# CCIG-Champalimaud/adell-mri

Hardware: AMD Instinct MI355X
Metric: volumes/sec 3D U-Net 128^3 2-ch seg (train step: fwd+loss+bwd+SGD) (higher is better)
Workload: dtype f32 (f16x3 split MFMA, fp32 accumulate); 1 GPU; BASELINE configs[1]: u-net-3d-resnet.yaml UNetPL, 2x128^3, batch 2/GPU, dice+focal, SGD-Nesterov; per_gpu_batch=2, parallelism=dp1, yaml=configs/u-net-3d-resnet.yaml, built_by=parse_config_unet -> get_segmentation_network('unet'), gradient_exchange=none (1 rank)

## Files before the change

adell_mri_amd/_lib.py:

```python
import ctypes
import os

_HERE = os.path.dirname(os.path.abspath(__file__))
LIB_PATH = os.environ.get("ADELL_HIP_LIBRARY") or os.path.join(_HERE, "libadellhip.so")

_lib = None

OK = 0
E_BADARG, E_UNSUPPORTED, E_HIP, E_NOMEM = -1, -2, -3, -4

ACT_IDS = {
    "identity": 0, "swish": 1, "silu": 1, "relu": 2, "leaky_relu": 3, "prelu": 4,
    "gelu": 5, "sigmoid": 6, "tanh": 7, "elu": 8,
}


class AdellHipError(RuntimeError):
    pass


class ConvDesc(ctypes.Structure):
    _fields_ = [(n, ctypes.c_int32) for n in (
        "N", "D", "H", "W", "C0", "C1", "Cout", "KD", "KH", "KW", "SD", "SH", "SW",
        "PD", "PH", "PW", "Do", "Ho", "Wo")]
# ... 96 lines not shown
    "adell_dice_focal_bwd_dev": (_i, [_vp, _vp, _i, _l, _f, _f, _f, _f, _f, _vp, _vp, _vp, _vp, _vp]),
    "adell_class_sums_workspace": (_l, [_i, _l, _i]),
    "adell_class_sums_fwd": (_i, [_vp, _vp, _i, _l, _i, _vp, _vp, ctypes.c_size_t, _vp]),
    "adell_class_sums_bwd": (_i, [_vp, _vp, _i, _l, _i, _vp, _vp]),
    "adell_sgd_step": (_i, [_vp, _vp, _vp, _l, _f, _f, _f, _i, _i, _f, _vp]),
    "adell_adamw_step": (_i, [_vp, _vp, _vp, _vp, _l, _f, _f, _f, _f, _f, _l, _f, _vp]),
    "adell_adam_step": (_i, [_vp, _vp, _vp, _vp, _l, _f, _f, _f, _f, _f, _l, _f, _vp]),
    "adell_ema_update": (_i, [_vp, _vp, _l, _f, _vp]),
    "adell_layernorm_fwd": (_i, [_vp, _vp, _vp, _vp, _vp, _vp, _l, _i, _f, _vp]),
    "adell_layernorm_bwd_workspace": (_l, [_l, _i]),
    "adell_layernorm_bwd": (_i, [_vp] * 8 + [_l, _i, _vp, ctypes.c_size_t, _vp]),
    "adell_add_bcast": (_i, [_vp, _vp, _vp, _l, _l, _vp]),
    "adell_sum_bcast": (_i, [_vp, _vp, _l, _l, _vp]),
    "adell_attention_fwd": (_i, [_vp, _vp, _vp, _vp, _i, _i, _i, _i, _i, _f, _f, ctypes.c_ulonglong,
                                 ctypes.c_uint, _vp, _vp, _vp]),
    "adell_attention_bwd": (_i, [_vp, _vp, _vp, _vp, _i, _vp, _vp, _vp, _i, _i, _i, _i, _f, _f,
                                 ctypes.c_ulonglong, ctypes.c_uint, _vp, _vp, _vp, _vp]),
    "adell_attention_strided_ok": (_i, [_i, _i, _i]),
    "adell_attention_plan": (_i, [_i] * 5 + [_vp]),
    "adell_attention_fwd_strided": (_i, [_vp, _vp, _vp, _vp, _i, _i, _i, _i, _i, _i, _vp, _f, _f,
                                         ctypes.c_ulonglong, ctypes.c_uint, _vp, _vp, _vp]),
    "adell_attention_bwd_strided": (_i, [_vp, _vp, _vp, _vp, _i, _vp, _vp, _vp, _i, _i, _i, _i, _i,
                                         _vp, _f, _f, ctypes.c_ulonglong, ctypes.c_uint, _vp, _vp,
                                         _vp, _vp]),
    "adell_attention_fwd_labels": (_i, [_vp, _vp, _vp, _vp, _i, _vp, _i, _i, _i, _i, _i, _i, _f, _f,
                                        ctypes.c_ulonglong, ctypes.c_uint, _vp, _vp, _vp]),
    "adell_attention_bwd_labels": (_i, [_vp, _vp, _vp, _vp, _i, _vp, _i, _i, _vp, _vp, _vp, _i, _i,
                                        _i, _i, _f, _f, ctypes.c_ulonglong, ctypes.c_uint, _vp, _vp,
                                        _vp, _vp]),
    "adell_attention_fwd_strided_labels": (_i, [_vp, _vp, _vp, _vp, _i, _vp, _i, _i, _i, _i, _i, _i,
                                                _vp, _f, _f, ctypes.c_ulonglong, ctypes.c_uint, _vp,
                                                _vp, _vp]),
    "adell_attention_bwd_strided_labels": (_i, [_vp, _vp, _vp, _vp, _i, _vp, _i, _vp, _vp, _vp, _i,
                                                _i, _i, _i, _i, _vp, _f, _f, ctypes.c_ulonglong,
                                                ctypes.c_uint, _vp, _vp, _vp, _vp]),
    "adell_attention_bias_grad_workspace_floats": (_l, [_i, _i]),
    "adell_attention_bias_grad": (_i, [_vp, _vp, _vp, _vp, _i, _vp, _i, _vp, _vp, _vp, _i, _i, _i,
                                       _i, _i, _vp, _f, _f, ctypes.c_ulonglong, ctypes.c_uint, _vp,
                                       _vp, _l, _vp]),
    "adell_copy_channels": (_i, [_vp, _vp, _l, _i, _i, _i, _i, _vp]),
    "adell_interp_nearest_fwd": (_i, [_vp, _vp] + [_i] * 8 + [_vp]),
    "adell_interp_nearest_bwd": (_i, [_vp, _vp] + [_i] * 8 + [_vp]),
    "adell_interp_linear_fwd": (_i, [_vp, _vp] + [_i] * 8 + [_f] * 3 + [_i, _vp]),
    "adell_interp_linear_bwd": (_i, [_vp, _vp] + [_i] * 8 + [_f] * 3 + [_i, _vp]),
    "adell_fold_x_taps": (_i, [_vp, _vp] + [_i] * 8 + [_vp]),
    "adell_scale_bc": (_i, [_vp, _vp, _vp, _i, _l, _i, _vp]),
    "adell_scale_bc_dscale_workspace_floats": (_l, [_i, _l, _i]),
    "adell_scale_bc_dscale": (_i, [_vp, _vp, _vp, _i, _l, _i, _vp, _vp]),
    "adell_cse_apply": (_i, [_vp, _vp, _vp, _vp, _vp, _vp, _i, _l, _i, _vp]),
    "adell_cse_apply_bwd_workspace_floats": (_l, [_i, _l, _i]),
    "adell_cse_apply_bwd": (_i, [_vp, _vp, _vp, _vp, _vp, _vp, _vp, _vp, _i, _l, _i, _vp, _vp]),
    "adell_bcast_nc": (_i, [_vp, _vp, _i, _l, _i, _f, _vp]),
    "adell_maxpool3d_fwd": (_i, [ctypes.POINTER(ConvDesc), _vp, _vp, _vp, _vp]),
    "adell_maxpool3d_bwd": (_i, [ctypes.POINTER(ConvDesc), _vp, _vp, _vp, _vp]),
    "adell_dwconv3d_fwd": (_i, [_i] * 8 + [_vp] * 5),
    "adell_dwconv3d_bwd_data": (_i, [_i] * 8 + [_vp] * 4),
    "adell_dwconv3d_bwd_weight_workspace_floats": (_l, [_i] * 8),
    "adell_dwconv3d_bwd_weight": (_i, [_i] * 8 + [_vp] * 6),
    "adell_vicreg_scratch_floats": (_l, [_i, _i]),
    "adell_vicreg_fwd": (_i, [_vp, _vp, _i, _i, _f, _f, _vp, _vp, _vp]),
    "adell_vicreg_bwd": (_i, [_vp, _vp, _i, _i, _f, _f, _vp, _vp, _vp, _vp, _vp]),
    "adell_convt_k2_applicable": (_i, [_i] * 6),
    "adell_convt_k2_fwd": (_i, [_i] * 6 + [_vp] * 5),
    "adell_convt_k2_bwd_data": (_i, [_i] * 6 + [_vp] * 4),
    "adell_convt_k2_wgrad_workspace": (_l, [_i] * 6),
    "adell_convt_k2_bwd_weight": (_i, [_i] * 6 + [_vp] * 5 + [ctypes.c_size_t, _vp]),
    "adell_convt_k221_applicable": (_i, [_i] * 6),
    "adell_convt_k221_fwd": (_i, [_i] * 6 + [_vp] * 5),
    "adell_convt_k221_bwd_data": (_i, [_i] * 6 + [_vp] * 4),
    "adell_convt_k221_wgrad_workspace": (_l, [_i] * 6),
    "adell_convt_k221_bwd_weight": (_i, [_i] * 6 + [_vp] * 5 + [ctypes.c_size_t, _vp]),
    "adell_conv_cinfold_applicable": (_i, [ctypes.POINTER(ConvDesc)]),
    "adell_conv_cinfold_ntiles": (_i, [ctypes.POINTER(ConvDesc)]),
    "adell_conv_cinfold_fwd": (_i, [ctypes.POINTER(ConvDesc)] + [_vp] * 5 + [_i, _vp]),
    "adell_conv_cinfold_fwd_f16x3": (_i, [ctypes.POINTER(ConvDesc)] + [_vp] * 5 + [_i, _vp]),
    "adell_conv_cinfold_wgrad_workspace": (_l, [ctypes.POINTER(ConvDesc)]),
    "adell_conv_cinfold_bwd_weight": (_i, [ctypes.POINTER(ConvDesc)] + [_vp] * 5
                                      + [ctypes.c_size_t, _vp]),
    "adell_conv_cinfold_bwd_weight_f16x3": (_i, [ctypes.POINTER(ConvDesc)] + [_vp] * 5
                                            + [ctypes.c_size_t, _vp]),
    "adell_conv_cinfold_dx_applicable": (_i, [ctypes.POINTER(ConvDesc)]),
    "adell_conv_cinfold_bwd_data": (_i, [ctypes.POINTER(ConvDesc)] + [_vp] * 4),
    "adell_conv_cinfold_bwd_data_f16x3": (_i, [ctypes.POINTER(ConvDesc)] + [_vp] * 4),
    "adell_pair_loss_scratch_floats": (_l, [_i, _i]),
    "adell_pair_loss_fwd": (_i, [_vp, _vp, _i, _i, _i, _f, _i, _vp, _vp, _vp]),
    "adell_pair_loss_bwd": (_i, [_vp, _vp, _i, _i, _i, _f, _i, _vp, _vp, _vp, _vp, _vp]),
    "adell_loco_loss_workspace": (_l, [_i, _l, _i]),
    "adell_loco_loss_fwd": (_i, [_vp, _vp, _i, _l, _i, _f, _f, _vp, _vp, ctypes.c_size_t, _vp]),
    "adell_loco_loss_bwd": (_i, [_vp, _vp, _vp, _i, _l, _i, _f, _f, _vp, _vp, _vp]),
    "adell_prelu_wgrad_workspace": (_l, [ctypes.POINTER(NormActDesc)]),
    "adell_prelu_wgrad": (_i, [ctypes.POINTER(NormActDesc)] + [_vp] * 8 + [ctypes.c_size_t, _vp]),
    "adell_convtranspose3d_fwd_f16x3": (_i, [_i] * 9 + [_vp] * 7),
    "adell_convtranspose3d_bwd_data_f16x3": (_i, [_i] * 9 + [_vp] * 6),
    "adell_convtranspose3d_f16x3_plan": (_i, [_i] * 9 + [_vp]),
    "adell_conv1_small_applicable": (_i, [ctypes.POINTER(ConvDesc)]),
    "adell_conv1_small_fwd": (_i, [ctypes.POINTER(ConvDesc)] + [_vp] * 6),
    "adell_conv1_small_bwd_data": (_i, [ctypes.POINTER(ConvDesc)] + [_vp] * 5),
    "adell_conv1_small_wgrad_workspace": (_l, [ctypes.POINTER(ConvDesc)]),
    "adell_conv1_small_bwd_weight": (_i, [ctypes.POINTER(ConvDesc)] + [_vp] * 6 + [ctypes.c_size_t, _vp]),
    "adell_conv_cin_small_applicable": (_i, [ctypes.POINTER(ConvDesc)]),
    "adell_conv_cin_small_ntiles": (_i, [ctypes.POINTER(ConvDesc)]),
    "adell_conv_cin_small_fwd": (_i, [ctypes.POINTER(ConvDesc)] + [_vp] * 5 + [_i, _vp]),
    "adell_conv_cin_small_bwd_data": (_i, [ctypes.POINTER(ConvDesc)] + [_vp] * 4),
    "adell_multi_copy": (_i, [_vp, _i, _vp, _vp]),
    "adell_grad_norm_workspace": (_l, [_i]),
    "adell_grad_norm_partials": (_i, [_vp, _l, _i, _vp, _i, _vp]),
    "adell_grad_norm_finalize": (_i, [_vp, _i, _i, _f, _f, _vp, _vp]),
    "adell_grad_scale_by": (_i, [_vp, _l, _vp, _vp]),
    "adell_multi_accumulate": (_i, [_vp, _i, _vp, _vp]),
    "adell_seg_confusion_workspace": (_l, [_l, _i]),
    "adell_seg_confusion_update": (_i, [_vp, _vp, _i, _l, _i, _l, _i, _vp, _l, _vp, _i, _vp]),
    "adell_seg_metric_compute": (_i, [_vp, _i, _i, _f, _vp, _vp]),
    "adell_cc_workspace": (_l, [_l, _i, _i, _i]),
    "adell_cc_label": (_i, [_vp, _l, _i, _i, _i, _i, _f, _vp, _vp, _vp, _l, _vp]),
    "adell_picai_tables_workspace": (_l, [_l, _i, _i, _i]),
    "adell_picai_tables_capacity": (_l, [_l, _i, _i, _i]),
    "adell_picai_tables": (_i, [_vp, _vp, _l, _i, _i, _i, _i, _f, _vp, _vp, _l, _vp, _l, _vp]),
    "adell_lesion_candidates_workspace": (_l, [_l, _i, _i, _i, _i]),
    "adell_lesion_candidates_capacity": (_l, [_i] * 6),
    "adell_lesion_candidates": (_i, [_vp, _l, _i, _i, _i, _i, _f, _f] + [_i] * 5 + [_vp] * 6
                                + [_l, ctypes.POINTER(ctypes.c_int), _vp, _l, _vp]),
    "adell_item_stats_workspace": (_l, [_i, _l]),
    "adell_item_stats": (_i, [_vp, _i, _l, _vp, _vp, ctypes.c_size_t, _vp]),
    "adell_aug_intensity": (_i, [_vp, _vp, _i, _l, _vp, ctypes.c_uint64, ctypes.c_uint32, _vp]),
    "adell_affine_sample": (_i, [_vp, _vp, _i, _i, _i, _i, _i, _vp, _i, _i, _vp]),
    "adell_axis_filter": (_i, [_vp, _vp, _i, _i, _i, _i, _i, _i, _vp, _i, _vp]),
    "adell_bias_field": (_i, [_vp, _vp, _i, _i, _i, _i, _i, _vp, _vp]),
    "adell_axis_lut_sample": (_i, [_vp, _vp, _i, _i, _i, _i, _i, _vp, _i, _vp]),
    "adell_dw_mfma_ok": (_i, [_i] * 8 + [_vp, _vp]),
    "adell_dw_dense_ok": (_i, [_i] * 8 + [_vp, _vp]),
    "adell_dw_wgrad_mfma_ok": (_i, [_i] * 8 + [_vp, _vp]),
    "adell_dwconv3d_plan": (_i, [_i] * 11 + [_vp]),
    "adell_wgrad_zring_plan": (_i, [_i] * 16 + [_vp]),
    "adell_rowscale_fwd": (_i, [_vp] * 5 + [_i, _i, _vp]),
    "adell_rowscale_bwd": (_i, [_vp] * 8 + [_i, _i, _vp]),
    "adell_window_ndhwc": (_i, [_vp, _vp] + [_i] * 11 + [_vp]),
    "adell_gibbs_workspace": (_l, [_i, _i, _i, _i, _i]),
    "adell_gibbs_lowpass": (_i, [_vp, _vp, _i, _i, _i, _i, _i, _vp, _vp, ctypes.c_size_t, _vp]),
    "adell_gather_nd": (_i, [_vp, _vp, _i, _vp, _vp, _vp, _i, _vp, _vp, _vp, _vp]),
    "adell_layernorm_rows_fwd": (_i, [_vp, _l, _i, _i, _l, _l, _vp, _vp, _f, _vp, _vp, _vp, _vp]),
    "adell_layernorm_rows_bwd_workspace": (_l, [_l, _i]),
    "adell_layernorm_rows_bwd": (_i, [_vp, _vp, _vp, _vp, _vp, _l, _i, _i, _l, _l, _vp, _l, _l,
                                      _vp, _vp, _vp, ctypes.c_size_t, _vp]),
    "adell_winattn_fwd": (_i, [_vp, _vp, _vp, _l, _l, _vp, _vp, _i, _l, _i, _i, _i, _i, _f, _f,
                               ctypes.c_ulong, ctypes.c_uint, _vp, _vp, _vp]),
    "adell_winattn_bwd": (_i, [_vp, _vp, _vp, _l, _l, _vp, _vp, _i, _vp, _vp, _vp, _l, _i, _i, _i,
                               _i, _f, _f, ctypes.c_ulong, ctypes.c_uint, _vp, _vp, _vp, _vp, _vp]),
    "adell_gemm_f32_workspace_floats": (_l, [_i, _i, _i]),
    "adell_gemm_f32": (_i, [_i, _i, _i, _vp, _l, _i, _vp, _l, _i, _vp, _l, _vp, _vp, _l, _vp, _vp]),
    "adell_absmax_f32": (_i, [_vp, _l, _vp, _vp]),
    "adell_gemm_f16x3_applicable": (_i, [_i, _i, _i, _vp, _l, _i, _vp, _l, _i]),
    "adell_gemm_f16x3_workspace_floats": (_l, [_i, _i, _i]),
    "adell_gemm_f16x3": (_i, [_i, _i, _i, _vp, _l, _i, _vp, _l, _i, _vp, _l, _vp, _vp, _l, _vp, _vp,
                              _vp, _vp]),
    "adell_gemm_f16x3_act": (_i, [_i, _i, _i, _vp, _l, _i, _vp, _l, _i, _vp, _l, _vp, _vp, _l, _vp,
                                  _vp, _vp, _i, _f, _vp, _vp, _vp]),
    "adell_optim_step": (_i, [_i, _vp, _vp, _vp, _vp, _l, _f, _f, _f, ctypes.POINTER(ctypes.c_float),
                              _vp]),
    "adell_seg_loss_workspace": (_l, [_i, _l, _i]),
    "adell_seg_loss_fwd": (_i, [_i, _vp, _vp, _vp, _i, _l, _i, _f, _f, _f, _f, _f, _f, _vp, _vp, _vp,
                                ctypes.c_size_t, _vp]),
    "adell_seg_loss_bwd": (_i, [_i, _vp, _vp, _vp, _i, _l, _i, _f, _f, _f, _f, _f, _f, _vp, _vp, _vp,
                                _vp]),
    "adell_channel_softmax_fwd": (_i, [_vp, _vp, _l, _i, _vp]),
    "adell_channel_softmax_bwd": (_i, [_vp, _vp, _vp, _l, _i, _vp]),
    "adell_channel_max_fwd": (_i, [_vp, _vp, _vp, _i, _l, _i, _vp]),
# ... 55 lines not shown
```

adell_mri_amd/csrc/conv_cinfold.hip:

```cpp
#include <type_traits>
#include "common.h"

struct CinFoldArgs {
  const float* x;
  const float* w;
  const float* bias;
  const float* dy;
  float* y;
  float* part;
  float* ws;
  int N, D, H, W, Cout, Do, Ho, Wo, PD, PH, PW;
  int ntx, nty, ntz;
};

template <int CIN>
struct CinFoldHalo {
  static constexpr int PER = (600 * CIN + 255) / 256;
  float v[PER];
  __device__ __forceinline__ void fetch(const CinFoldArgs& a, int nb, int ox0, int oy0, int oz0) {
#pragma unroll
    for (int u = 0; u < PER; ++u) {
      const int i = threadIdx.x + 256 * u;
      const int ci = i % CIN, hv = i / CIN;
      const int hx = hv % 10, hy = (hv / 10) % 10, hz = hv / 100;
// ... 1137 lines not shown
          for (int kx = 0; kx < 3; ++kx) {
            const int r = (vy + 2 - ky) * 10 + (vx + 2 - kx);
            t9 += sT[r * TS + ((kz * 3 + ky) * 3 + kx) * CIN + ci];
          }
        run[kz] += t9;
      }
      const int z = p - a.PD, yy = y0 + vy, xx = x0 + vx;
      if (z >= z_beg && z < z_end && yy < a.H && xx < a.W)
        a.dx[((((size_t)nb * a.D + z) * a.H + yy) * a.W + xx) * CIN + ci] = run[0];
      run[0] = run[1];
      run[1] = run[2];
      run[2] = 0.f;
    }
  }
}

extern "C" int adell_conv_cinfold_dx_applicable(const adell_conv3d_desc* d) {
  return (adell_cinfold_ok(d) && d->Cout <= 64 && d->Cout % 4 == 0) ? 1 : 0;
}

template <int CIN, int CO>
static int adell_cinfold_dx_f16_launch(const CinFoldDxArgs& a, dim3 grid, hipStream_t st) {
  constexpr int KP = ((27 * CIN + 31) / 32) * 32;
  const size_t lds = (size_t)((CO / 16) * 128 * 16 + 128 * (KP + 1) + 8) * sizeof(float);
  return adell_launch<adell_cinfold_dx_f16_kernel<CIN, CO>>(grid, dim3(256), lds, st, a);
}

template <int CIN>
static int adell_cinfold_dx_launch(const CinFoldDxArgs& a, dim3 grid, hipStream_t st, int f16x3) {
  constexpr int KP = ((27 * CIN + 31) / 32) * 32;
  if (f16x3 && a.Cout <= 32) return adell_cinfold_dx_f16_launch<CIN, 32>(a, grid, st);
  if constexpr (CIN < 4) {
    if (f16x3) return adell_cinfold_dx_f16_launch<CIN, 64>(a, grid, st);
  }
  if (a.Cout <= 32) {
    const size_t lds = (size_t)(128 * 33 + 128 * (KP + 1)) * sizeof(float);
    return adell_launch<adell_cinfold_dx_kernel<CIN, 32>>(grid, dim3(256), lds, st, a);
  }
  const size_t lds = (size_t)(128 * 65 + 128 * (KP + 1)) * sizeof(float);
  return adell_launch<adell_cinfold_dx_kernel<CIN, 64>>(grid, dim3(256), lds, st, a);
}

static int adell_cinfold_bwd_data_impl(const adell_conv3d_desc* d, const float* dy, const float* w,
                                       float* dx, int f16x3, void* stream);

extern "C" int adell_conv_cinfold_bwd_data(const adell_conv3d_desc* d, const float* dy,
                                           const float* w, float* dx, void* stream) {
  return adell_cinfold_bwd_data_impl(d, dy, w, dx, 0, stream);
}

extern "C" int adell_conv_cinfold_bwd_data_f16x3(const adell_conv3d_desc* d, const float* dy,
                                                 const float* w, float* dx, void* stream) {
  return adell_cinfold_bwd_data_impl(d, dy, w, dx, 1, stream);
}

static int adell_cinfold_bwd_data_impl(const adell_conv3d_desc* d, const float* dy, const float* w,
                                       float* dx, int f16x3, void* stream) {
  ADELL_REQUIRE(dy && w && dx && adell_conv_cinfold_dx_applicable(d),
                "conv_cinfold_bwd_data: 3x3x3 stride-1 conv, 1..4 input channels, Cout <= 64 "
                "(multiple of 4) expected");
  ADELL_REQUIRE((((uintptr_t)dy) & 15) == 0, "conv_cinfold_bwd_data: dy must be 16-byte aligned");
  CinFoldDxArgs a = {};
  a.dy = dy; a.w = w; a.dx = dx;
  a.N = d->N; a.D = d->D; a.H = d->H; a.W = d->W; a.Cout = d->Cout;
  a.Do = d->Do; a.Ho = d->Ho; a.Wo = d->Wo; a.PD = d->PD; a.PH = d->PH; a.PW = d->PW;
  a.ntx = adell_cdiv(d->W, 8);
  a.nty = adell_cdiv(d->H, 8);
  const long cols = (long)a.ntx * a.nty * d->N;
  int nseg = (int)((512 + cols - 1) / cols);
  if (nseg < 1) nseg = 1;
  while (nseg > 1 && adell_cdiv(d->D, nseg) < 8) --nseg;
  a.nseg = nseg;
  a.seglen = adell_cdiv(d->D, nseg);
  a.nseg = adell_cdiv(d->D, a.seglen);
  dim3 grid((unsigned)(a.ntx * a.nty * a.nseg), (unsigned)d->N);
  hipStream_t st = (hipStream_t)stream;
  switch (d->C0) {
    case 1: return adell_cinfold_dx_launch<1>(a, grid, st, f16x3);
    case 2: return adell_cinfold_dx_launch<2>(a, grid, st, f16x3);
    case 3: return adell_cinfold_dx_launch<3>(a, grid, st, f16x3);
    default: return adell_cinfold_dx_launch<4>(a, grid, st, f16x3);
  }
}
```

adell_mri_amd/csrc/norm_act.hip:

```cpp
#include "common.h"

ADELL_RNG_STEP_DEFINE(norm_act)

__global__ __launch_bounds__(256) void adell_stats_finalize_kernel(
    const float* __restrict__ part, int N, int ntiles, int C, double count, float eps,
    int per_item, float* __restrict__ mean, float* __restrict__ rstd) {
  __shared__ double sh[8][32][2];
  const int cl = threadIdx.x & 31, sl = threadIdx.x >> 5;
  const int c = blockIdx.x * 32 + cl;
  const int nbeg = per_item ? blockIdx.y : 0, nend = per_item ? blockIdx.y + 1 : N;
  double s1 = 0.0, s2 = 0.0;
  if (c < C) {
    for (int n = nbeg; n < nend; ++n) {
      const float* p = part + ((size_t)n * ntiles * C + c) * 2;
      int t = sl;
      for (; t + 56 < ntiles; t += 64) {
        float2 v[8];
#pragma unroll
        for (int u = 0; u < 8; ++u)
          v[u] = *reinterpret_cast<const float2*>(p + (size_t)(t + 8 * u) * C * 2);
#pragma unroll
        for (int u = 0; u < 8; ++u) {
          s1 += (double)v[u].x;
          s2 += (double)v[u].y;
        }
      }
      for (; t < ntiles; t += 8) {
        const float2 v = *reinterpret_cast<const float2*>(p + (size_t)t * C * 2);
        s1 += (double)v.x;
        s2 += (double)v.y;
      }
    }
  }
  sh[sl][cl][0] = s1;
  sh[sl][cl][1] = s2;
  __syncthreads();
  if (sl == 0 && c < C) {
    double a = 0.0, b = 0.0;
#pragma unroll
    for (int k = 0; k < 8; ++k) {
      a += sh[k][cl][0];
      b += sh[k][cl][1];
    }
    const double cnt = per_item ? count : count * N;
    const double m = a / cnt;
    double var = b / cnt - m * m;
    if (var < 0.0) var = 0.0;
    const size_t o = per_item ? (size_t)blockIdx.y * C + c : (size_t)c;
    mean[o] = (float)m;
    rstd[o] = (float)(1.0 / sqrt(var + (double)eps));
  }
}

__global__ __launch_bounds__(256) void adell_stats_fold_kernel(const float* __restrict__ part,
                                                               int ntiles, int C, int Z,
                                                               float* __restrict__ out,
                                                               int pstride, int poff) {
  __shared__ double sh[8][32][2];
  const int cl = threadIdx.x & 31, sl = threadIdx.x >> 5;
  const int c = blockIdx.x * 32 + cl, n = blockIdx.y, z = blockIdx.z;
  const int t0 = z * 256;
  const int t1 = t0 + 256 < ntiles ? t0 + 256 : ntiles;
  double s1 = 0.0, s2 = 0.0;
  if (c < C) {
    const float* p = part + ((size_t)n * ntiles * pstride + poff + c) * 2;
    int t = t0 + sl;
    for (; t + 56 < t1; t += 64) {
      float2 v[8];
#pragma unroll
      for (int u = 0; u < 8; ++u)
        v[u] = *reinterpret_cast<const float2*>(p + (size_t)(t + 8 * u) * pstride * 2);
#pragma unroll
      for (int u = 0; u < 8; ++u) {
        s1 += (double)v[u].x;
        s2 += (double)v[u].y;
      }
    }
    for (; t < t1; t += 8) {
      const float2 v = *reinterpret_cast<const float2*>(p + (size_t)t * pstride * 2);
      s1 += (double)v.x;
      s2 += (double)v.y;
    }
  }
// ... 832 lines not shown

static void adell_na_bwd_partials_launch(NormActBwdArgs& a, const adell_norm_act_desc* d, bool fast,
                                         bool vec, hipStream_t st) {
  dim3 grid(a.ntiles, (unsigned)d->N);
  if (fast) {
    a.ntiles = (int)adell_na_fast_blocks(d->V, d->C);
    if (a.lr_g) {
      ADELL_ACT_DISPATCH_LR(adell_na_bwd_partials_fast_kernel, d->act,
                            dim3(a.ntiles, (unsigned)d->N), st, a);
    } else {
      ADELL_ACT_DISPATCH(adell_na_bwd_partials_fast_kernel, d->act,
                         dim3(a.ntiles, (unsigned)d->N), st, a);
    }
  } else if (vec)
    hipLaunchKernelGGL(adell_na_bwd_partials_kernel<true>, grid, dim3(256), 0, st, a);
  else
    hipLaunchKernelGGL(adell_na_bwd_partials_kernel<false>, grid, dim3(256), 0, st, a);
}

static void adell_na_bwd_apply_launch(const NormActBwdArgs& a, const adell_norm_act_desc* d,
                                      bool fast, bool vec, hipStream_t st) {
  const long nw = vec ? a.total / 4 : a.total;
  if (fast) {
    long bx = ((a.VC >> 2) + 256 * ADELL_EW_UNROLL - 1) / (256 * ADELL_EW_UNROLL);
    if (bx > ADELL_EW_MAXBLOCKS) bx = ADELL_EW_MAXBLOCKS;
    if (bx < 1) bx = 1;
    if (a.lr_g) {
      ADELL_ACT_DISPATCH_LR(adell_na_bwd_apply_fast_kernel, d->act,
                            dim3((unsigned)bx, (unsigned)d->N), st, a);
    } else {
      ADELL_ACT_DISPATCH(adell_na_bwd_apply_fast_kernel, d->act,
                         dim3((unsigned)bx, (unsigned)d->N), st, a);
    }
  } else if (vec)
    hipLaunchKernelGGL(adell_na_bwd_apply_kernel<true>, dim3(adell_ew_blocks(nw)), dim3(256), 0,
                       st, a);
  else
    hipLaunchKernelGGL(adell_na_bwd_apply_kernel<false>, dim3(adell_ew_blocks(nw)), dim3(256),
                       0, st, a);
}

static int adell_norm_act_bwd_impl(const adell_norm_act_desc* d, const float* x,
                                   const float* dout, const float* mean, const float* rstd,
                                   const float* gamma, const float* beta, const float* act_w,
                                   float* dx, float* dgamma, float* dbeta, void* workspace,
                                   size_t workspace_bytes, void* stream, const float* lr_g,
                                   const float* lr_w, int lr_co) {
  NormActBwdArgs a = {};
  int rc = adell_nab_fill(&a, d);
  if (rc != ADELL_OK) return rc;
  a.lr_g = lr_g; a.lr_w = lr_w; a.lr_co = lr_co;
  a.lr_shift = adell_ilog2(d->C) - 2;
  ADELL_REQUIRE(x && dout && dx, "norm_act_bwd: null pointer");
  ADELL_REQUIRE((mean == nullptr) == (rstd == nullptr), "norm_act_bwd: mean/rstd mismatch");
  hipStream_t st = (hipStream_t)stream;
  a.x = x; a.dout = dout; a.mean = mean; a.rstd = rstd; a.gamma = gamma; a.beta = beta;
  a.act_w = act_w; a.dx = dx;
  bool vec, fast;
  adell_na_bwd_route(a, d, &vec, &fast);
  if (mean || dgamma || dbeta) {
    ADELL_REQUIRE(workspace && (long)workspace_bytes >= adell_norm_act_bwd_workspace(d),
                  "norm_act_bwd: workspace too small");
    float* part = (float*)workspace;
    long ntmax = a.ntiles;
    if (adell_na_fast_blocks(d->V, d->C) > ntmax) ntmax = adell_na_fast_blocks(d->V, d->C);
    float* c1 = part + (size_t)d->N * ntmax * d->C * 2;
    float* c2 = c1 + (size_t)d->N * d->C;
    a.part = part; a.c1 = c1; a.c2 = c2;
    adell_na_bwd_partials_launch(a, d, fast, vec, st);
    if (d->stats_per_item && !dgamma && !dbeta && d->N <= 65535)
      hipLaunchKernelGGL(adell_na_bwd_finalize_item_kernel,
                         dim3(adell_cdiv(d->C, 8), (unsigned)d->N), dim3(256), 0, st,
                         (const float*)part, a.ntiles, d->C, (double)d->V, gamma, c1, c2, d->C, 0);
    else
      hipLaunchKernelGGL(adell_na_bwd_finalize_kernel, dim3(adell_cdiv(d->C, 32)), dim3(1024), 0,
                         st, (const float*)part, (int)d->N, a.ntiles, d->C, (double)d->V,
                         d->stats_per_item, gamma, c1, c2, dgamma, dbeta);
  }
  adell_na_bwd_apply_launch(a, d, fast, vec, st);
  ADELL_CHECK_HIP(hipGetLastError());
  return ADELL_OK;
}

struct NaConst {
  float m[4], r[4], g[4], b[4], p[4], c1[4], c2[4];
};

__device__ __forceinline__ void adell_na_consts(NaConst& k, const float* mean, const float* rstd,
                                                const float* gamma, const float* beta,
                                                const float* act_w, int act_w_n, float act_p,
                                                const float* c1, const float* c2, long sbase,
                                                int c, int cmask) {
#pragma unroll
  for (int j = 0; j < 4; ++j) {
    const int cj = (c + j) & cmask;
    k.m[j] = mean ? mean[sbase + cj] : 0.f;
    k.r[j] = rstd ? rstd[sbase + cj] : 1.f;
    k.g[j] = gamma ? gamma[cj] : 1.f;
    k.b[j] = beta ? beta[cj] : 0.f;
    k.p[j] = act_w ? act_w[act_w_n > 1 ? cj : 0] : act_p;
    k.c1[j] = c1 ? c1[sbase + cj] : 0.f;
    k.c2[j] = c2 ? c2[sbase + cj] : 0.f;
  }
}

struct NaLowRank {
  float w[4][4];
};
__device__ __forceinline__ void adell_na_lr_load(NaLowRank& l, const NormActBwdArgs& a, int c) {
#pragma unroll
  for (int o = 0; o < 4; ++o)
#pragma unroll
    for (int q = 0; q < 4; ++q)
      l.w[o][q] = o < a.lr_co ? a.lr_w[o * a.C + c + q] : 0.f;
}
__device__ __forceinline__ float4 adell_na_lr_dout(const NaLowRank& l, const NormActBwdArgs& a,
                                                   int n, long jj) {
  const float* g = a.lr_g + ((long)n * a.V + (jj >> a.lr_shift)) * a.lr_co;
  float4 r = make_float4(0.f, 0.f, 0.f, 0.f);
#pragma unroll
  for (int o = 0; o < 4; ++o)
    if (o < a.lr_co) {
      const float gv = g[o];
      r.x = fmaf(gv, l.w[o][0], r.x); r.y = fmaf(gv, l.w[o][1], r.y);
      r.z = fmaf(gv, l.w[o][2], r.z); r.w = fmaf(gv, l.w[o][3], r.w);
    }
  return r;
}

template <int ACT>
__global__ __launch_bounds__(256) void adell_norm_act_fwd_fast_kernel(NormActArgs a) {
  const int n = a.rev ? (int)(gridDim.y - 1 - blockIdx.y) : (int)blockIdx.y;
  const long n4 = a.VC >> 2;
  ADELL_EW_RANGE(n4);
  const int c = (int)((j0 << 2) & (a.C - 1));
  NaConst k;
  adell_na_consts(k, a.mean, a.rstd, a.gamma, a.beta, a.act_w, a.act_w_n, a.act_p, nullptr,
                  nullptr, (long)n * a.stat_stride_n, c, a.C - 1);
  const float keep_scale = a.drop_p > 0.f ? 1.0f / (1.0f - a.drop_p) : 1.0f;
  const float4* xin = reinterpret_cast<const float4*>(a.x) + (long)n * n4;
  float4* yout = reinterpret_cast<float4*>(a.out) + (long)n * n4;
  for (long j = j0; j < jend; j += stride * ADELL_EW_UNROLL) {
    float4 v[ADELL_EW_UNROLL];
#pragma unroll
    for (int u = 0; u < ADELL_EW_UNROLL; ++u)
      if (j + u * stride < jend) v[u] = xin[j + u * stride];
#pragma unroll
    for (int u = 0; u < ADELL_EW_UNROLL; ++u) {
      const long jj = j + u * stride;
      if (jj >= jend) break;
      float h[4] = {v[u].x, v[u].y, v[u].z, v[u].w};
      uint32_t rr[4] = {0, 0, 0, 0};
      if (a.drop_p > 0.f) {
        const long gi = (long)n * n4 + jj;
        const uint4 r = adell_philox4((uint32_t)gi, (uint32_t)(gi >> 32), a.rng_offset + g_adell_rng_step, 0u,
                                      a.seed_lo, a.seed_hi);
        rr[0] = r.x; rr[1] = r.y; rr[2] = r.z; rr[3] = r.w;
      }
      bool kept[4] = {true, true, true, true};
#pragma unroll
      for (int q = 0; q < 4; ++q) {
        float t = ((h[q] - k.m[q]) * k.r[q]) * k.g[q] + k.b[q];
        if (a.drop_p > 0.f) {
          const float uu = (float)(rr[q] >> 8) * (1.0f / 16777216.0f);
          kept[q] = uu >= a.drop_p;
          t = kept[q] ? t * keep_scale : 0.f;
        }
        h[q] = adell_act_fwd(ACT, t, k.p[q]);
      }
      if (a.split) {
        na_half4 hi, lo;
#pragma unroll
        for (int q = 0; q < 4; ++q) {
          const float t = __builtin_amdgcn_fmed3f(h[q] * a.split_scale, -65504.f, 65504.f);
          const _Float16 hh = (_Float16)t;
          hi[q] = hh;
          lo[q] = (_Float16)(t - (float)hh);
        }
        const int within = (int)((jj << 2) & 15);
        char* row = reinterpret_cast<char*>(a.out) + 4 * ((long)n * a.VC + (jj << 2) - within);
        *reinterpret_cast<na_half4*>(row + within * 2) = hi;
        *reinterpret_cast<na_half4*>(row + 32 + within * 2) = lo;
      } else {
        yout[jj] = make_float4(h[0], h[1], h[2], h[3]);
      }
      if (a.mask != nullptr) {
        unsigned long long b[4];
#pragma unroll
        for (int q = 0; q < 4; ++q) b[q] = __ballot(kept[q]);
        const int ln = threadIdx.x & 63;
        if (ln < 4)
          a.mask[((long)n * a.groups + (jj >> 6)) * 4 + ln] =
              ln == 0 ? b[0] : (ln == 1 ? b[1] : (ln == 2 ? b[2] : b[3]));
      }
    }
  }
}

template <int ACT, bool LR>
__global__ __launch_bounds__(256) void adell_na_bwd_apply_fast_kernel(NormActBwdArgs a) {
  const int n = blockIdx.y;
  const long n4 = a.VC >> 2;
  ADELL_EW_RANGE(n4);
  const int c = (int)((j0 << 2) & (a.C - 1));
  NaConst k;
  adell_na_consts(k, a.mean, a.rstd, a.gamma, a.beta, a.act_w, a.act_w_n, a.act_p, a.c1, a.c2,
                  (long)n * a.stat_stride_n, c, a.C - 1);
  const float keep_scale = a.drop_p > 0.f ? 1.0f / (1.0f - a.drop_p) : 1.0f;
  const float4* xin = reinterpret_cast<const float4*>(a.x) + (long)n * n4;
  const float4* gin = reinterpret_cast<const float4*>(a.dout) + (long)n * n4;
  float4* dxo = reinterpret_cast<float4*>(a.dx) + (long)n * n4;
  const bool norm = a.mean != nullptr;
  NaLowRank lr;
  if (LR) adell_na_lr_load(lr, a, c);
  for (long j = j0; j < jend; j += stride * ADELL_EW_UNROLL) {
    float4 xv[ADELL_EW_UNROLL], gv[ADELL_EW_UNROLL];
#pragma unroll
    for (int u = 0; u < ADELL_EW_UNROLL; ++u)
      if (j + u * stride < jend) {
        xv[u] = xin[j + u * stride];
        gv[u] = LR ? adell_na_lr_dout(lr, a, n, j + u * stride) : gin[j + u * stride];
      }
#pragma unroll
    for (int u = 0; u < ADELL_EW_UNROLL; ++u) {
      const long jj = j + u * stride;
      if (jj >= jend) break;
      const float xs[4] = {xv[u].x, xv[u].y, xv[u].z, xv[u].w};
      const float gs[4] = {gv[u].x, gv[u].y, gv[u].z, gv[u].w};
      bool keep[4];
      adell_na_keep4(a, (long)n * n4 + jj, keep);
      float o[4];
#pragma unroll
      for (int q = 0; q < 4; ++q) {
        const float hn = (xs[q] - k.m[q]) * k.r[q];
        const float t = hn * k.g[q] + k.b[q];
        const float uu = keep[q] ? t * keep_scale : 0.f;
        const float du = gs[q] * adell_act_grad(ACT, uu, k.p[q]);
        const float dt = keep[q] ? du * keep_scale : 0.f;
        float r = dt * k.g[q];
        if (norm) r = k.r[q] * (r - k.c1[q] - hn * k.c2[q]);
        o[q] = r;
      }
      dxo[jj] = make_float4(o[0], o[1], o[2], o[3]);
    }
  }
}

template <int ACT, bool LR>
__global__ __launch_bounds__(256) void adell_na_bwd_partials_fast_kernel(NormActBwdArgs a) {
  __shared__ float sh[8][256];
  const int n = blockIdx.y;
  const long n4 = a.VC >> 2;
  ADELL_EW_RANGE(n4);
  const int c = (int)((j0 << 2) & (a.C - 1));
  NaConst k;
  adell_na_consts(k, a.mean, a.rstd, a.gamma, a.beta, a.act_w, a.act_w_n, a.act_p, nullptr,
                  nullptr, (long)n * a.stat_stride_n, c, a.C - 1);
  const float keep_scale = a.drop_p > 0.f ? 1.0f / (1.0f - a.drop_p) : 1.0f;
  const float4* xin = reinterpret_cast<const float4*>(a.x) + (long)n * n4;
  const float4* gin = reinterpret_cast<const float4*>(a.dout) + (long)n * n4;
  float A[4] = {0.f, 0.f, 0.f, 0.f}, B[4] = {0.f, 0.f, 0.f, 0.f};
  NaLowRank lr;
  if (LR) adell_na_lr_load(lr, a, c);
  for (long j = j0; j < jend; j += stride * ADELL_EW_UNROLL) {
    float4 xv[ADELL_EW_UNROLL], gv[ADELL_EW_UNROLL];
#pragma unroll
    for (int u = 0; u < ADELL_EW_UNROLL; ++u)
      if (j + u * stride < jend) {
        xv[u] = xin[j + u * stride];
        gv[u] = LR ? adell_na_lr_dout(lr, a, n, j + u * stride) : gin[j + u * stride];
      }
#pragma unroll
    for (int u = 0; u < ADELL_EW_UNROLL; ++u) {
      const long jj = j + u * stride;
      if (jj >= jend) break;
      const float xs[4] = {xv[u].x, xv[u].y, xv[u].z, xv[u].w};
      const float gs[4] = {gv[u].x, gv[u].y, gv[u].z, gv[u].w};
      bool keep[4];
      adell_na_keep4(a, (long)n * n4 + jj, keep);
#pragma unroll
      for (int q = 0; q < 4; ++q) {
        const float hn = (xs[q] - k.m[q]) * k.r[q];
        const float t = hn * k.g[q] + k.b[q];
        const float uu = keep[q] ? t * keep_scale : 0.f;
        const float du = gs[q] * adell_act_grad(ACT, uu, k.p[q]);
        const float dt = keep[q] ? du * keep_scale : 0.f;
        A[q] += dt;
        B[q] += dt * hn;
      }
    }
  }
#pragma unroll
  for (int q = 0; q < 4; ++q) {
    sh[q][threadIdx.x] = A[q];
    sh[4 + q][threadIdx.x] = B[q];
  }
  __syncthreads();
  if (a.C < 4) {
    if (threadIdx.x < 2 * a.C) {
      const int ch = threadIdx.x % a.C, which = threadIdx.x / a.C;
      float s1 = 0.f;
      for (int kk = 0; kk < 256; ++kk)
        for (int q = ch; q < 4; q += a.C) s1 += sh[which * 4 + q][kk];
      a.part[(((size_t)n * a.ntiles + blockIdx.x) * a.C + ch) * 2 + which] = s1;
    }
    return;
  }
  const int CG = a.C >> 2;
  const int VL = CG >= 256 ? 1 : 256 / CG;
  const int nout = (CG < 256 ? CG : 256) * 8;
  for (int o = threadIdx.x; o < nout; o += 256) {
    const int cl = o % (nout / 8), q8 = o / (nout / 8);
    float s1 = 0.f;
    for (int kk = 0; kk < VL; ++kk) s1 += sh[q8][kk * CG + cl];
    const int quad = (int)(((jbeg + cl) << 2) & (a.C - 1));
    const int ch = quad + (q8 & 3);
    a.part[(((size_t)n * a.ntiles + blockIdx.x) * a.C + ch) * 2 + (q8 >> 2)] = s1;
  }
}


__global__ __launch_bounds__(256) void adell_na_bwd_apply_dt_kernel(NormActBwdArgs a) {
  const int n = blockIdx.y;
  const long n4 = a.VC >> 2;
  ADELL_EW_RANGE(n4);
  const int c = (int)((j0 << 2) & (a.C - 1));
  NaConst k;
  adell_na_consts(k, a.mean, a.rstd, nullptr, nullptr, nullptr, 0, 0.f, a.c1, a.c2,
                  (long)n * a.stat_stride_n, c, a.C - 1);
  const float4* xin = reinterpret_cast<const float4*>(a.x) + (long)n * n4;
  const float4* gin = reinterpret_cast<const float4*>(a.dout) + (long)n * n4;
  float4* dxo = reinterpret_cast<float4*>(a.dx) + (long)n * n4;
  for (long j = j0; j < jend; j += stride * ADELL_EW_UNROLL) {
    float4 xv[ADELL_EW_UNROLL], gv[ADELL_EW_UNROLL];
#pragma unroll
    for (int u = 0; u < ADELL_EW_UNROLL; ++u)
      if (j + u * stride < jend) {
        xv[u] = xin[j + u * stride];
        gv[u] = gin[j + u * stride];
      }
#pragma unroll
    for (int u = 0; u < ADELL_EW_UNROLL; ++u) {
      const long jj = j + u * stride;
      if (jj >= jend) break;
      const float xs[4] = {xv[u].x, xv[u].y, xv[u].z, xv[u].w};
      const float gs[4] = {gv[u].x, gv[u].y, gv[u].z, gv[u].w};
      float o[4];
#pragma unroll
      for (int q = 0; q < 4; ++q) {
        const float hn = (xs[q] - k.m[q]) * k.r[q];
        o[q] = k.r[q] * (gs[q] - k.c1[q] - hn * k.c2[q]);
      }
      dxo[jj] = make_float4(o[0], o[1], o[2], o[3]);
    }
  }
}

extern "C" int adell_norm_act_bwd_from_dt(const adell_norm_act_desc* d, const float* x,
                                          const float* dt, const float* mean, const float* rstd,
                                          const float* partials, int ntiles, int pstride, int poff,
                                          float* dx, void* workspace, size_t workspace_bytes,
                                          void* stream) {
  NormActBwdArgs a = {};
  int rc = adell_nab_fill(&a, d);
  if (rc != ADELL_OK) return rc;
  ADELL_REQUIRE(x && dt && dx && mean && rstd && partials && workspace,
                "norm_act_bwd_from_dt: null pointer");
  ADELL_REQUIRE(d->stats_per_item == 1 && d->N <= 65535,
                "norm_act_bwd_from_dt: instance statistics only");
// ... 355 lines not shown
```

adell_mri_amd/functional.py:

```python
import itertools
import os
import weakref

import numpy as np
import torch
import torch.distributed as dist

from . import _lib, ops

_dropout_counter = itertools.count(1)

CONV_PRECISION = os.environ.get("ADELL_CONV_PRECISION", "f16x3")
FLAGS = {"s2class_always": bool(os.environ.get("ADELL_S2CLASS_ALWAYS")),
         "no_s2class": bool(os.environ.get("ADELL_NO_S2CLASS")),
         "no_fold": bool(os.environ.get("ADELL_NO_FOLD")),
         "no_adn_fuse": bool(os.environ.get("ADELL_NO_ADN_FUSE")),
         "no_lowrank": bool(os.environ.get("ADELL_NO_LOWRANK")),
         "wgrad_stream": os.environ.get("ADELL_WGRAD_STREAM", "1") != "0",
         "no_rows": bool(os.environ.get("ADELL_NO_ROWS")),
         "no_pointwise_gemm": bool(os.environ.get("ADELL_NO_POINTWISE_GEMM")),
         "no_seq_attention": bool(os.environ.get("ADELL_NO_SEQ_ATTENTION")),
         "no_mlp_fuse": not bool(os.environ.get("ADELL_MLP_FUSE")),
         "mlp_min_elems": int(os.environ.get("ADELL_MLP_MIN_ELEMS", str(1 << 20))),
         "no_cinfold_wgrad_f16": bool(os.environ.get("ADELL_NO_CINFOLD_WGRAD_F16"))}


def set_conv_precision(mode):
    global CONV_PRECISION
    if mode not in ("f16x3", "fp32"):
        raise ValueError("conv precision must be 'f16x3' or 'fp32'")
    CONV_PRECISION = mode
    _sync_dw_precision()


def _sync_dw_precision():
    from . import _lib
    if os.path.exists(_lib.LIB_PATH) and not os.environ.get("ADELL_DW_NOMFMA"):
        _lib.lib().adell_set_tuning(b"dw_nomfma", 1 if CONV_PRECISION == "fp32" else 0)


if CONV_PRECISION == "fp32":
    _sync_dw_precision()


class _Ref:

    __slots__ = ("obj",)

    def __init__(self, obj):
        self.obj = obj


_PACK_REG = {}
_PACK_BATCH = {"epoch": -1, "sig": None, "table": None, "blocks": 0}


class _PackFence:

    __slots__ = ("stream", "event")

    def __init__(self):
        self.stream = ops._stream().value
        self.event = torch.cuda.Event()
        self.event.record()

    def order(self):
        if ops._stream().value != self.stream:
            torch.cuda.current_stream().wait_event(self.event)


def _pack_tag(w):
    return (w._version, w.data_ptr(), ops.WEIGHT_EPOCH)


def _repack_registered():
    live = []
    for key, ent in list(_PACK_REG.items()):
        w = ent[0]()
        if w is None or not w.is_contiguous() or not w.is_cuda:
            del _PACK_REG[key]
            continue
        live.append((w, ent))
    if not live:
        return False
    rows, first = [], 0
    for w, ent in live:
        d0, d1 = w.shape[0], w.shape[1]
        taps = w.shape[2] * w.shape[3] * w.shape[4]
        rows.append((w.data_ptr(), ent[2].halfs.data_ptr(), ent[2].scale.data_ptr(), ent[1], d0,
                     d1, taps, first))
        first += d0 if ent[1] == 0 else d1
    sig = tuple(rows)
    if _PACK_BATCH["sig"] != sig and torch.cuda.is_current_stream_capturing():
        return False
    if _PACK_BATCH["sig"] != sig:
        _PACK_BATCH["table"] = torch.tensor(rows, dtype=torch.int64, device=live[0][0].device)
        _PACK_BATCH["sig"] = sig
        _PACK_BATCH["blocks"] = first
    ops.pack_weight_f16x3_multi(_PACK_BATCH["table"], len(rows), _PACK_BATCH["blocks"])
    fence = _PackFence()
    for w, ent in live:
        ent[3] = _pack_tag(w)
        ent[4] = fence
    _PACK_BATCH["epoch"] = ops.WEIGHT_EPOCH
    return True


# ... 220 lines not shown
    return True


_ROWS_EXPECT = weakref.WeakKeyDictionary()
_ROWS_PLAN = {}


def _hooked(producers, readers):
    gm = torch.nn.modules.module
    if gm._global_forward_hooks or gm._global_forward_pre_hooks:
        return True
    for top in producers:
        for m in top.modules():
            if m._forward_hooks:
                return True
    for top in readers:
        for m in top.modules():
            if m._forward_pre_hooks:
                return True
    return False


def expect_rows(adn_module, conv, as_x1=False, producers=(), readers=()):
    spec = conv.rows_spec() if (not FLAGS["no_rows"] and hasattr(conv, "rows_spec")) else None
    if spec is not None and _hooked((adn_module,) + tuple(producers), (conv,) + tuple(readers)):
        spec = None
    if spec is None:
        _ROWS_EXPECT.pop(adn_module, None)
    else:
        _ROWS_EXPECT[adn_module] = spec + (bool(as_x1),)


def clear_row_expectations():
    if _ROWS_EXPECT:
        _ROWS_EXPECT.clear()


def take_rows_reader(adn_module):
    return _ROWS_EXPECT.pop(adn_module, None) if _ROWS_EXPECT else None


def _rows_exponent(x, reader, norm, gamma, beta, act, act_p, act_w, p):
    if (reader is None or FLAGS["no_rows"] or CONV_PRECISION != "f16x3" or norm != "instance"
            or p >= 1.0
            or gamma is not None or beta is not None or act_w is not None or x.dim() != 5
            or act not in ("identity", "swish", "silu", "relu", "leaky_relu", "gelu")
            or (act == "leaky_relu" and abs(act_p) > 1.0)):
        return None
    weight, stride, padding, as_x1 = reader
    N, C = x.shape[:2]
    spatial = tuple(x.shape[2:])
    other = weight.shape[1] - C
    if weight.dim() != 5 or other < 0 or C < 16 or (C & (C - 1)) or C > 1024:
        return None
    C0, C1 = (other, C) if as_x1 else (C, other)
    if C0 == 0:
        C0, C1 = C1, 0
    grad = torch.is_grad_enabled() and weight.requires_grad
    key = (N, spatial, C0, C1, tuple(weight.shape), stride, padding, grad, ops.plan_epoch())
    ok = _ROWS_PLAN.get(key)
    if ok is None:
        k = tuple(weight.shape[2:])
        ok = ops.conv3d_rows_ok(N, spatial, C0, C1, weight.shape[0], k, stride, padding)
        if ok and grad:
            ok = ops.conv3d_bwd_weight_rows_ok(N, spatial, C0, C1, weight.shape[0], k, stride,
                                               padding)
        _ROWS_PLAN[key] = ok
    if not ok:
        return None
    V = spatial[0] * spatial[1] * spatial[2]
    bound = float(np.sqrt(V)) / (1.0 - p)
    return 14 - int(np.ceil(np.log2(max(bound, 1.0))))


def materialize(t):
    rows = getattr(t, "_adell_rows", None)
    return t if rows is None else ops.rows_to_f32(t.detach(), rows)


class _Conv3dFn(torch.autograd.Function):
    @staticmethod
    def forward(ctx, x0, x1, weight, bias, residual, wp, conf):
        (stride, padding, want_stats, wref, ctx.carry_in, ctx.carry_out, ctx.carry_x0,
         ctx.carry_cat, ctx.adn, rows0, rows1) = conf
        if (rows0 is not None or rows1 is not None) and not isinstance(wp, ops.SplitWeight):
            ops.ROWS_FALLBACKS[0] += 1
            if rows0 is not None:
                x0, rows0 = ops.rows_to_f32(x0, rows0), None
            if rows1 is not None:
                x1, rows1 = ops.rows_to_f32(x1, rows1), None
        ctx.rows = (rows0, rows1)
        k = tuple(weight.shape[2:]) if weight.dim() == 5 else (1, 1, 1)
        ctx.set_materialize_grads(False)
        ctx.bias_ref = _Ref(bias)
        ctx.cin_small = wp == "cin_small"
        ctx.cinfold = wp == "cinfold"
        if ctx.cinfold:
            y, part = ops.conv_cinfold_fwd(x0, weight, bias, padding, want_stats,
                                           f16x3=CONV_PRECISION == "f16x3")
            ctx.small1 = False
            ctx.amax = None
            ctx.save_for_backward(x0, x1, weight)
            ctx.conf = (k, stride, padding, bias is not None, False, wref)
            if part is None:
                part = y.new_empty(0)
            ctx.mark_non_differentiable(part)
            return y, part
        if ctx.cin_small:
            y, part = ops.conv_cin_small_fwd(x0, weight, bias, padding, want_stats)
            ctx.small1 = False
            ctx.amax = None
            ctx.save_for_backward(x0, x1, weight)
            ctx.conf = (k, stride, padding, bias is not None, False, wref)
            if part is None:
                part = y.new_empty(0)
            ctx.mark_non_differentiable(part)
            return y, part
        if isinstance(wp, tuple) and wp[0] == "fold":
            xf = ops.fold_x_taps(x0, k[2], padding[2])
            y, part = ops.conv3d_fwd(xf, wp[1], bias, weight.shape[0], (k[0], k[1], 1), stride,
                                     (padding[0], padding[1], 0), residual=residual,
                                     want_stats=want_stats)
            ctx.small1 = False
            ctx.amax = None
            ctx.save_for_backward(x0, x1, weight)
            ctx.conf = (k, stride, padding, bias is not None, residual is not None, wref)
            if part is None:
                part = y.new_empty(0)
            ctx.mark_non_differentiable(part)
            return y, part
        ctx.small1 = wp is None
        if ctx.small1:
            y = ops.conv1_small_fwd(x0, x1, weight, bias)
            ctx.save_for_backward(x0, x1, weight)
            ctx.conf = (k, stride, padding, bias is not None, False, wref)
            part = y.new_empty(0)
            ctx.mark_non_differentiable(part)
            return y, part
        amax = None
        if isinstance(wp, ops.SplitWeight) and ctx.needs_input_grad[2]:
            amax = _amax_pair(x0.device)
        y, part = ops.conv3d_fwd(x0, wp, bias, weight.shape[0], k, stride, padding, x1=x1,
                                 residual=residual, want_stats=want_stats,
                                 amax=None if amax is None else amax[0:1], rows0=rows0, rows1=rows1)
        ctx.amax = amax
        ctx.save_for_backward(x0, x1, weight)
        ctx.conf = (k, stride, padding, bias is not None, residual is not None, wref)
        if part is None:
            part = y.new_empty(0)
        ctx.mark_non_differentiable(part)
        return y, part

    @staticmethod
    def backward(ctx, dy, _dpart):
        x0, x1, weight = ctx.saved_tensors
        k, stride, padding, has_bias, has_res, wref = ctx.conf
        need = ctx.needs_input_grad
        if dy is None:
            _side_ok(wref.obj)
            add0 = ctx.carry_in.take() if ctx.carry_in is not None else None
            return (add0 if need[0] else None), None, None, None, None, None, None
        dy = ops.ndhwc(dy)
        dx0 = dx1 = dw = db = dres = None
        add0 = ctx.carry_in.take() if ctx.carry_in is not None else None
        C0 = x0.shape[1]
        C1 = 0 if x1 is None else x1.shape[1]
        if ctx.small1:
            if ctx.adn is not None and need[0]:
                ctx.adn[1].lowrank = (dy, weight.detach())
                dx0 = dy.new_zeros(()).expand(x0.shape)
            elif need[0] or (x1 is not None and need[1]):
                dx0, dx1 = ops.conv1_small_bwd_data(dy, weight, tuple(x0.shape[2:]), C0, C1)
                dx0 = dx0 if need[0] else None
                dx1 = dx1 if (x1 is not None and need[1]) else None
            if need[2] or (has_bias and need[3]):
                if _side_ok(wref.obj, ctx.bias_ref.obj):
                    dw, db = side_run(lambda: ops.conv1_small_bwd_weight(
                        x0, x1, dy, has_bias and need[3]), (x0, x1, dy))
                else:
                    dw, db = ops.conv1_small_bwd_weight(x0, x1, dy, has_bias and need[3])
                dw = dw.view(weight.shape) if need[2] else None
            if add0 is not None and dx0 is not None:
                dx0 = dx0 + add0
            dx0, dx1 = _park_input_grads(ctx, dx0, dx1)
            return dx0, dx1, dw, db, None, None, None
        amax = ctx.amax
        dy_amax = None
        if getattr(ctx, "cinfold", False) and need[0]:
            dx0 = ops.conv_cinfold_bwd_data(dy, weight, tuple(x0.shape[2:]), padding,
                                            f16x3=CONV_PRECISION == "f16x3")
        if dx0 is not None:
            pass
        elif ctx.cin_small and need[0] and dy.shape[1] % 4 == 0:
            dx0 = ops.conv_cin_small_bwd_data(dy, weight, tuple(x0.shape[2:]), padding)
        elif (ctx.cin_small and need[0] and dy.shape[1] <= 4 and stride == (1, 1, 1)
              and tuple(dy.shape[2:]) == tuple(x0.shape[2:])):
            wt = weight.detach().transpose(0, 1).flip(2, 3, 4).contiguous()
            pt = tuple(kk - 1 - pp for kk, pp in zip(k, padding))
            dx0, _ = ops.conv_cin_small_fwd(dy, wt, None, pt, False)
        elif (need[0] and x1 is None and CONV_PRECISION == "f16x3"
              and ops.conv3d_bwd_data_s2_fused_ok(x0.shape[2:], C0, C1, dy.shape[1], k, stride,
                                                  padding)
              and isinstance(_packed(wref.obj, 1), ops.SplitWeight)):
            if amax is not None:
                dy_amax = amax[1:2]
            dx0 = ops.conv3d_bwd_data_s2_fused(dy, _packed(wref.obj, 1), tuple(x0.shape[2:]),
                                               amax=dy_amax, add0=add0)
            add0 = None
        elif (need[0] and x1 is None and CONV_PRECISION == "f16x3" and stride == (2, 2, 2)
              and k == (3, 3, 3) and all(p <= 1 for p in padding)
              and all(s % 2 == 0 for s in x0.shape[2:])
              and (x0.numel() // C0 >= (1 << 20) or FLAGS["s2class_always"])
              and not FLAGS["no_s2class"]):
            if amax is not None:
                dy_amax = amax[1:2]
            dx0 = ops.conv3d_bwd_data_s2(dy, _packed_s2_classes(wref.obj, padding),
                                         tuple(x0.shape[2:]), C0, padding, amax=dy_amax,
                                         add0=add0)
            add0 = None
        elif (ctx.adn is not None and need[0] and (x1 is None or need[1])
              and (add0 is None or C1 == 0) and isinstance(_packed(wref.obj, 1), ops.SplitWeight)):
            site0, site1, ntiles, epoch = ctx.adn
            wpb = _packed(wref.obj, 1)
            if amax is not None:
                dy_amax = amax[1:2]
            if epoch != ops.plan_epoch():
                ntiles = ops.conv3d_bwd_data_adn_ntiles(tuple(x0.shape[2:]), x0.shape[0], C0, C1,
                                                        dy.shape[1], k, stride, padding)
            if ntiles > 0:
                dx0, dx1, part = ops.conv3d_bwd_data_adn(dy, wpb, tuple(x0.shape[2:]), C0, C1, k,
                                                         stride, padding, ntiles, site0=site0,
                                                         site1=site1, amax=dy_amax, add0=add0)
                add0 = None
                if site0 is not None:
                    site0.fused, site0.part, site0.poff = True, part, 0
                if site1 is not None:
                    site1.fused, site1.part, site1.poff = True, part, C0
            else:
                fused = add0 is not None and C1 == 0
                dx0, dx1 = ops.conv3d_bwd_data(dy, wpb, tuple(x0.shape[2:]), C0, C1, k, stride,
                                               padding, amax=dy_amax, add0=add0 if fused else None)
                if fused:
                    add0 = None
                if x1 is None or not need[1]:
                    dx1 = None
        elif need[0] or (x1 is not None and need[1]):
            wpb = _packed(wref.obj, 1)
            if amax is not None and isinstance(wpb, ops.SplitWeight):
                dy_amax = amax[1:2]
            fused = add0 is not None and C1 == 0 and isinstance(wpb, ops.SplitWeight)
            dx0, dx1 = ops.conv3d_bwd_data(dy, wpb, tuple(x0.shape[2:]), C0, C1, k, stride,
                                           padding, amax=dy_amax, add0=add0 if fused else None)
            if fused:
                add0 = None
            if not need[0]:
                dx0 = None
            if x1 is None or not need[1]:
                dx1 = None
        want_db = has_bias and need[3]

        def weight_grads():
            dw = db = None
            if need[2] and getattr(ctx, "cinfold", False):
                dw, db = ops.conv_cinfold_bwd_weight(
                    x0, dy, padding, want_db,
                    f16x3=(CONV_PRECISION == "f16x3" and not FLAGS["no_cinfold_wgrad_f16"]))
                dw = dw.view(weight.shape)
            elif need[2]:
                rows0, rows1 = getattr(ctx, "rows", (None, None))
                dw = ops.conv3d_bwd_weight(x0, dy, k, stride, padding, x1=x1, want_db=want_db,
                                           f16x3=(CONV_PRECISION == "f16x3"),
                                           x_amax=None if amax is None else amax[0:1],
                                           dy_amax=dy_amax, rows0=rows0, rows1=rows1)
                if want_db:
                    dw, db = dw
                dw = dw.view(weight.shape)
            elif want_db:
                db = ops.bias_grad(dy)
            return dw, db

        if (need[2] or want_db) and _side_ok(wref.obj, ctx.bias_ref.obj):
            dw, db = side_run(weight_grads, (x0, x1, dy))
        else:
            dw, db = weight_grads()
        if add0 is not None and dx0 is not None:
            dx0 = dx0 + add0
        dx0, dx1 = _park_input_grads(ctx, dx0, dx1)
        if has_res and need[4]:
            if ctx.carry_out is not None:
                ctx.carry_out.grad = dy
            else:
                dres = dy
        return dx0, dx1, dw, db, dres, None, None


def _park_input_grads(ctx, dx0, dx1):
    if dx0 is not None and ctx.carry_x0 is not None:
        ctx.carry_x0.grad, dx0 = dx0, None
    if dx1 is not None and ctx.carry_cat is not None:
        ctx.carry_cat.grad, dx1 = dx1, None
    return dx0, dx1


def grad_observed(t):
    return bool(getattr(t, "_backward_hooks", None)) or bool(getattr(t, "retains_grad", False))


class GradCarry:

    __slots__ = ("grad",)

    def __init__(self):
        self.grad = None

    def take(self):
        g, self.grad = self.grad, None
        return g


class AdnSite:

    __slots__ = ("x", "mean", "rstd", "mask", "drop_p", "act", "act_p", "fused", "part", "poff",
                 "lowrank")

    def __init__(self, x, mean, rstd, mask, drop_p, act, act_p):
        self.x, self.mean, self.rstd, self.mask = x, mean, rstd, mask
        self.drop_p, self.act, self.act_p = drop_p, act, act_p
        self.fused, self.part, self.poff = False, None, 0
        self.lowrank = None


def single_use(t):
    if t is not None and getattr(t, "_adell_site", None) is not None:
        t._adell_single = True
    return t


_ADN_PLAN = {}


def _adn_sites_of(x0, x1, weight, stride, padding):
    s0 = (getattr(x0, "_adell_site", None)
          if getattr(x0, "_adell_single", False) and not grad_observed(x0) else None)
    s1 = (getattr(x1, "_adell_site", None)
          if x1 is not None and getattr(x1, "_adell_single", False) and not grad_observed(x1)
          else None)
    if (s0 is None and s1 is None) or CONV_PRECISION != "f16x3" or FLAGS["no_adn_fuse"] \
            or weight.dim() != 5 or not torch.is_grad_enabled():
        return None
    C0 = x0.shape[1]
    C1 = 0 if x1 is None else x1.shape[1]
    key = (tuple(x0.shape), C1, tuple(weight.shape), stride, padding, ops.plan_epoch())
    nt = _ADN_PLAN.get(key)
    if nt is None:
        nt = ops.conv3d_bwd_data_adn_ntiles(tuple(x0.shape[2:]), x0.shape[0], C0, C1,
                                            weight.shape[0], tuple(weight.shape[2:]), stride,
                                            padding)
        _ADN_PLAN[key] = nt
    if nt <= 0:
        return None
    return (s0, s1, nt, key[-1])


def conv3d(x0, weight, bias=None, stride=1, padding=0, x1=None, residual=None, want_stats=True,
           carry_in=None, carry_out=None, carry_x0=None, carry_cat=None):
    stride, padding = ops._triple(stride), ops._triple(padding)
    if (weight.dim() == 5 and tuple(weight.shape[2:]) == (1, 1, 1) and stride == (1, 1, 1)
            and padding == (0, 0, 0) and x1 is None and residual is None and carry_in is None
            and carry_out is None and carry_x0 is None and carry_cat is None and x0.dim() == 5
            and getattr(x0, "_adell_rows", None) is None and max(weight.shape[:2]) >= 64
            and min(weight.shape[:2]) >= 8 and not FLAGS["no_pointwise_gemm"]):
        xr = ops.ndhwc(x0)
        N, C, D, H, W = xr.shape
        y2 = linear(xr.permute(0, 2, 3, 4, 1).reshape(-1, C), weight.view(weight.shape[0], C), bias)
        return y2.view(N, D, H, W, -1).permute(0, 4, 1, 2, 3)
    _note_use(weight)
    adn = _adn_sites_of(x0, x1, weight, stride, padding)
    rows0 = getattr(x0, "_adell_rows", None)
    rows1 = getattr(x1, "_adell_rows", None) if x1 is not None else None
    conf = (stride, padding, want_stats, _Ref(weight), carry_in, carry_out, carry_x0, carry_cat,
            adn, rows0, rows1)
    Cin = x0.shape[1] + (0 if x1 is None else x1.shape[1])
    small1 = ops.conv1_small_ok(weight, Cin, stride, padding, residual)
    if small1:
        wp = None
        site = getattr(x0, "_adell_site", None) if getattr(x0, "_adell_single", False) else None
        if (site is not None and x1 is None and carry_in is None and carry_x0 is None
                and not grad_observed(x0)
                and not FLAGS["no_adn_fuse"] and not FLAGS["no_lowrank"]
                and torch.is_grad_enabled() and ops.norm_act_lowrank_ok(x0, weight.shape[0])):
            conf = conf[:8] + (("lowrank", site),) + conf[9:]
    elif ops.conv_cin_small_ok(weight, x0, x1, stride, padding, residual):
        wp = "cin_small"
    elif ops.conv_cinfold_ok(weight, x0, x1, stride, padding, residual):
        wp = "cinfold"
    elif (CONV_PRECISION == "f16x3" and x1 is None and weight.dim() == 5 and x0.shape[1] <= 4
          and 3 <= weight.shape[4] and weight.shape[4] * x0.shape[1] <= 16
          and stride == (1, 1, 1) and not FLAGS["no_fold"]):
        wp = ("fold", _packed_folded(weight))
    else:
        wp = _packed(weight, 0)
    y, part = _Conv3dFn.apply(x0, x1, weight, bias, residual, wp, conf)
    if want_stats and part.numel() > 0:
        y._adell_partials = part
    return y


class _ConvT3dFn(torch.autograd.Function):
    @staticmethod
    def forward(ctx, x, weight, bias, wp, wref):
        factors = tuple(weight.shape[2:])
        ctx.k2 = wp is None
        if ctx.k2:
            y = ops.convt_k2_fwd(x, weight, bias)
        else:
            y = ops.convtranspose3d_fwd(x, wp, bias, weight.shape[1], factors)
        ctx.save_for_backward(x, weight)
        ctx.has_bias = bias is not None
        ctx.bias_ref = _Ref(bias)
        ctx.wref = wref
        ctx.factors = factors
        return y

    @staticmethod
    def backward(ctx, dy):
        x, weight = ctx.saved_tensors
        need = ctx.needs_input_grad
        dy = ops.ndhwc(dy)
        dx = dw = db = None
        if need[0]:
            dx = (ops.convt_k2_bwd_data(dy, weight) if ctx.k2 else
                  ops.convtranspose3d_bwd_data(dy, _packed(ctx.wref.obj, 3), weight.shape[0],
                                               ctx.factors))
        want_db = ctx.has_bias and need[2]

        def weight_grads():
            dw = db = None
            if need[1] and ctx.k2 and want_db:
                dw, db = ops.convt_k2_bwd_weight(x, dy, want_db=True, factors=ctx.factors)
            elif need[1]:
                dw = (ops.convt_k2_bwd_weight(x, dy, factors=ctx.factors) if ctx.k2 else
                      ops.convtranspose3d_bwd_weight(x, dy, ctx.factors))
            if want_db and db is None:
                db = ops.bias_grad(dy)
            return dw, db

        if (need[1] or want_db) and _side_ok(ctx.wref.obj, ctx.bias_ref.obj):
            dw, db = side_run(weight_grads, (x, dy))
        else:
            dw, db = weight_grads()
        return dx, dw, db, None, None


def conv_transpose3d(x, weight, bias=None):
    wp = None if (x.dim() == 5 and ops.convt_k2_ok(x.shape, weight)) else _packed(weight, 2)
    _note_use(weight)
    return _ConvT3dFn.apply(x, weight, bias, wp, _Ref(weight))


conv_transpose3d_k2s2 = conv_transpose3d


class _NormDropActFn(torch.autograd.Function):
    @staticmethod
    def forward(ctx, x, mean, rstd, gamma, beta, act_w, conf):
        act, act_p, per_item, drop_p, seed, offset, site, split_exp, _group = conf
        if site is not None:
            out, mask = ops.norm_act_fwd(x, mean, rstd, act, gamma=gamma, beta=beta, act_w=act_w,
                                         act_p=act_p, stats_per_item=per_item, drop_p=drop_p,
                                         seed=seed, rng_offset=offset, want_mask=True,
                                         split_exp=split_exp)
            site.x, site.mean, site.rstd, site.mask = x, mean, rstd, mask
        else:
            out = ops.norm_act_fwd(x, mean, rstd, act, gamma=gamma, beta=beta, act_w=act_w,
                                   act_p=act_p, stats_per_item=per_item, drop_p=drop_p, seed=seed,
                                   rng_offset=offset, split_exp=split_exp)
        ctx.save_for_backward(x, mean, rstd, gamma, beta, act_w)
        ctx.conf = conf
        return out

    @staticmethod
    def backward(ctx, dout):
        x, mean, rstd, gamma, beta, act_w = ctx.saved_tensors
        act, act_p, per_item, drop_p, seed, offset, site, _split_exp, group = ctx.conf
        if site is not None:
            fused, part, poff = site.fused, site.part, site.poff
            site.fused, site.part = False, None
            lowrank, site.lowrank = site.lowrank, None
            site.x = site.mean = site.rstd = site.mask = None
            if lowrank is not None:
                dx = ops.norm_act_bwd_lowrank(x, lowrank[0], lowrank[1], mean, rstd, act,
                                              act_p=act_p, drop_p=drop_p, seed=seed,
                                              rng_offset=offset)
                return dx, None, None, None, None, None, None
            if fused:
                dx = ops.norm_act_bwd_from_dt(x, ops.ndhwc(dout), mean, rstd, part, poff)
                return dx, None, None, None, None, None, None
        dact_w = None
        if act_w is not None and ctx.needs_input_grad[5]:
            dact_w = ops.prelu_wgrad(x, dout, mean, rstd, act_w, gamma=gamma, beta=beta,
                                     stats_per_item=per_item, drop_p=drop_p, seed=seed,
                                     rng_offset=offset)
        want_affine = gamma is not None and (ctx.needs_input_grad[3] or ctx.needs_input_grad[4])
        if group is not None:
            rec, dgamma, dbeta = ops.norm_act_bwd_sums(
                x, dout, mean, rstd, act, gamma=gamma, beta=beta, act_w=act_w, act_p=act_p,
                drop_p=drop_p, seed=seed, rng_offset=offset, want_affine_grads=want_affine)
            dist.all_reduce(rec, op=dist.ReduceOp.SUM, group=group)
            dx = ops.norm_act_bwd_apply_sums(x, dout, mean, rstd, rec, act, gamma=gamma, beta=beta,
                                             act_w=act_w, act_p=act_p, drop_p=drop_p, seed=seed,
                                             rng_offset=offset)
            if beta is None:
                dbeta = None
            return dx, None, None, dgamma, dbeta, dact_w, None
        dx, dgamma, dbeta = ops.norm_act_bwd(
            x, dout, mean, rstd, act, gamma=gamma, beta=beta, act_w=act_w, act_p=act_p,
            stats_per_item=per_item, drop_p=drop_p, seed=seed, rng_offset=offset,
            want_affine_grads=want_affine)
        if beta is None:
            dbeta = None
        return dx, None, None, dgamma, dbeta, dact_w, None


def norm_drop_act(x, *, norm="none", eps=1e-5, gamma=None, beta=None, running=None,
                  momentum=0.1, act="identity", act_p=0.0, act_w=None, drop_p=0.0,
                  training=False, rows_reader=None, sync_group=None):
    part = getattr(x, "_adell_partials", None)
    x = ops.ndhwc(x)
    N, C = x.shape[:2]
    V = x.shape[2] * x.shape[3] * x.shape[4]
    mean = rstd = group = None
    per_item = 1
    if norm == "instance":
        if part is None:
            part = ops.channel_partials(x.detach())
        mean, rstd = ops.stats_finalize(part, V, eps, per_item=True)
    elif norm == "batch":
        per_item = 0
        if (training and sync_group is not None
                and dist.get_world_size(group=sync_group) > 1):
            if part is None:
                part = ops.channel_partials(x.detach())
            rec = ops.bn_stats_sums(part, V)
            dist.all_reduce(rec, op=dist.ReduceOp.SUM, group=sync_group)
            mean, rstd = ops.bn_stats_from_sums(rec, eps, running, momentum)
            group = sync_group
        elif training or running is None or running[0] is None:
            if part is None:
                part = ops.channel_partials(x.detach())
            mean, rstd = ops.stats_finalize(part, V, eps, per_item=False)
            if training and running is not None and running[0] is not None:
                rm, rv, nbt = running
                if nbt is None and momentum is None:
                    raise ValueError("BatchNorm with momentum=None needs num_batches_tracked")
                ops.bn_running_update(mean, rstd, rm, rv, nbt, N * V, eps, momentum)
        else:
            rstd_c = torch.rsqrt(running[1] + eps)
            gamma = rstd_c if gamma is None else rstd_c * gamma
            shift = -running[0] * gamma
            beta = shift if beta is None else beta + shift
    elif norm != "none":
        raise NotImplementedError(f"norm {norm!r} has no HIP kernel yet")
    p = float(drop_p) if training else 0.0
    seed, offset = 0, 0
    if p > 0.0:
        seed = torch.initial_seed()
        offset = next(_dropout_counter)
    site = None
    if (norm == "instance" and gamma is None and beta is None and act_w is None
            and act in ("identity", "swish", "silu", "relu", "leaky_relu") and x.requires_grad
            and torch.is_grad_enabled() and not FLAGS["no_adn_fuse"] and CONV_PRECISION == "f16x3"
            and ops.norm_act_mask_ok(x)):
        site = AdnSite(None, None, None, None, p, act, float(act_p))
    split_exp = _rows_exponent(x, rows_reader, norm, gamma, beta, act, float(act_p), act_w, p)
    conf = (act, float(act_p), per_item, p, seed, offset, site, split_exp, group)
    out = _NormDropActFn.apply(x, mean, rstd, gamma, beta, act_w, conf)
    if site is not None:
        out._adell_site = site
    if split_exp is not None:
        out._adell_rows = ops.SplitRows(split_exp, ops.split_exponents(N, C, split_exp, x.device))
    return out


def _rows_as_volume(x):
    x = x.contiguous()
    C = x.shape[-1]
    return x.view(1, 1, 1, -1, C).permute(0, 4, 1, 2, 3)


def _volume_as_rows(y, lead_shape):
    C = y.shape[1]
    return y.permute(0, 2, 3, 4, 1).reshape(*lead_shape, C)


class _LinearFn(torch.autograd.Function):

    @staticmethod
    def forward(ctx, x, weight, bias, residual):
        N, K = weight.shape
        x2 = x.reshape(-1, K).contiguous()
        rows = x2.shape[0]
        w = weight.contiguous()
        res2 = None if residual is None else residual.reshape(rows, N).contiguous()
        split = CONV_PRECISION == "f16x3" and ops.gemm_f16x3_ok(rows, N, K, x2, K, True, w, K, True)
        if split:
            y = ops.gemm_f16x3(rows, N, K, x2, K, True, w, K, True, bias=bias, residual=res2)
        else:
            y = ops.gemm(rows, N, K, x2, K, True, w, K, True, bias=bias, residual=res2)
        ctx.save_for_backward(x2, w)
        ctx.split = split
        ctx.refs = (_Ref(weight), _Ref(bias))
        ctx.meta = (x.shape, bias is not None, residual is not None and residual.shape)
        return y.view(*x.shape[:-1], N)

    @staticmethod
    def backward(ctx, dy):
        x2, w = ctx.saved_tensors
        xshape, has_bias, res_shape = ctx.meta
        split = ctx.split
        N, K = w.shape
        rows = x2.shape[0]
        need = ctx.needs_input_grad
        dy2 = dy.reshape(rows, N).contiguous()
        dx = dw = db = dres = None
        if need[0]:
            if split and ops.gemm_f16x3_ok(rows, K, N, dy2, N, True, w, K, False):
                dx = ops.gemm_f16x3(rows, K, N, dy2, N, True, w, K, False)
            else:
                dx = ops.gemm(rows, K, N, dy2, N, True, w, K, False)
            dx = dx.view(xshape)
        def weight_grads():
            dw = db = None
            if need[1]:
                if split and ops.gemm_f16x3_ok(N, K, rows, dy2, N, False, x2, K, False):
                    dw = ops.gemm_f16x3(N, K, rows, dy2, N, False, x2, K, False)
                else:
                    dw = ops.gemm(N, K, rows, dy2, N, False, x2, K, False)
            if has_bias and need[2]:
                db = ops.bias_grad(_rows_as_volume(dy2))
            return dw, db

        if (need[1] or (has_bias and need[2])) and _side_ok(ctx.refs[0].obj, ctx.refs[1].obj):
            dw, db = side_run(weight_grads, (x2, dy2))
        else:
            dw, db = weight_grads()
        if res_shape and need[3]:
            dres = dy2.view(res_shape)
        return dx, dw, db, dres


class _MlpFn(torch.autograd.Function):

    @staticmethod
    def forward(ctx, x, w1, b1, w2, b2, residual, act, act_p):
        H, K = w1.shape
        N = w2.shape[0]
        x2 = x.reshape(-1, K).contiguous()
        rows = x2.shape[0]
# ... 789 lines not shown
```

adell_mri_amd/modules/segmentation/unet.py:

```python
from typing import Dict, List

import numpy as np
import torch

from ... import functional as HF
from ... import ops
from ..._lib import AdellHipError
from ..layers.adn_fn import ActDropNorm, get_adn_fn, norm_fn_dict
from ..layers.conv import (Conv2d, Conv3d, ConvTranspose2d, ConvTranspose3d, MaxPool2d,
                           MaxPool3d, Upsample)
from ..layers.linear_blocks import Linear
from ..layers.regularization import UOut
from ..layers.res_blocks import (DepthwiseConv2dStrided, DepthwiseConv3dStrided, ResidualBlock2d,
                                 ResidualBlock3d)
from ..layers.utils import crop_to_size


def _per_dim(v, n):
    return [v for _ in range(n)] if isinstance(v, int) else list(v)


class ConcatConvBlock(torch.nn.Sequential):

    def forward(self, X, X_cat=None, carry_cat=None):
        mods = list(self)
        if X_cat is not None and carry_cat is not None and _takes_carry(mods[0]):
            h = mods[0](X, X_cat=X_cat, carry_cat=carry_cat)
        else:
            h = mods[0](X, X_cat=X_cat) if X_cat is not None else mods[0](X)
        return _run_rest(mods[1:], h)


def _run_rest(mods, h):
    for i, mod in enumerate(mods):
        only_reader = (isinstance(mod, ActDropNorm) and i + 1 < len(mods)
                       and type(mods[i + 1]) is Conv3d)
        if only_reader:
            HF.expect_rows(mod, mods[i + 1])
        h = mod(h)
        if only_reader:
            h = HF.single_use(h)
    return h


def _last_adn(module):
    if isinstance(module, ResidualBlock3d):
        adn = getattr(module, "adn_op", None)
        return adn if isinstance(adn, ActDropNorm) and module.skip_activation is not True else None
    if isinstance(module, _DecoderOp) and len(module) > 0 and isinstance(module[-1], ActDropNorm):
        return module[-1]
    return None


def _first_conv(module):
    while isinstance(module, torch.nn.Sequential) and len(module) > 0:
        module = module[0]
    return module if type(module) is Conv3d else None


def _takes_carry(module):
    return type(module) is Conv3d and module.takes_carry()


def _head_with_carry(module, X, **carries):
    if _takes_carry(module):
        return module(X, **carries)
    if isinstance(module, torch.nn.Sequential) and len(module) > 0:
        mods = list(module)
        h = _head_with_carry(mods[0], X, **carries)
        if h is not None:
            for mod in mods[1:]:
                h = mod(h)
        return h
    return None


def _cat_channels(a, b):
    if a.dim() == 4:
        return HF.cat_channels([a.unsqueeze(2), b.unsqueeze(2)]).squeeze(2)
    return HF.cat_channels([a, b])


def _nearest(x, size):
    if x.dim() == 4:
        return HF.interpolate_nearest(x.unsqueeze(2), (1, *size)).squeeze(2)
    return HF.interpolate_nearest(x, size)


class SaeBlock(torch.nn.Sequential):

    def forward(self, X, X_cat=None, carry_cat=None):
        h = self[0](X, X_cat=X_cat, carry_cat=carry_cat) if X_cat is not None else self[0](X)
        return self[1](h)


class _DecoderOp(torch.nn.Sequential):

    def forward(self, X, X_cat=None, carry_cat=None):
        mods = list(self)
        if X_cat is not None and isinstance(mods[0], (ConcatConvBlock, SaeBlock)):
            h = mods[0](X, X_cat=X_cat, carry_cat=carry_cat)
        else:
            h = mods[0](X if X_cat is None else _cat_channels(X, X_cat))
        for mod in mods[1:]:
            h = mod(h)
        return h


def _keep_arguments(module, arguments: dict, skip=("self", "parent_class")):
    for name, value in arguments.items():
        if name not in skip and not name.startswith("__"):
            setattr(module, name, value)


class UNet(torch.nn.Module):
    def __init__(self, spatial_dimensions: int = 2,
                 encoding_operations: List[torch.nn.ModuleList] = None,
                 conv_type: str = "regular", link_type: str = "identity",
                 upscale_type: str = "upsample", interpolation: str = "bilinear",
                 norm_type: str = "batch", dropout_type: str = "dropout", padding: str = "same",
                 dropout_param: float = 0.1, activation_fn: torch.nn.Module = torch.nn.PReLU,
                 in_channels: int = 1, n_classes: int = 2, depth: list = [16, 32, 64],
                 kernel_sizes: list = [3, 3, 3], strides: list = [2, 2, 2],
                 bottleneck_classification: bool = False, skip_conditioning: int = None,
                 feature_conditioning: int = None,
                 feature_conditioning_params: Dict[str, torch.Tensor] = None,
                 deep_supervision: bool = False, parent_class: bool = False,
                 encoder_only: bool = False):
        arguments = dict(locals())
        super().__init__()
        _keep_arguments(self, arguments)

        if self.encoder_only is True or parent_class is False:
            self.get_norm_op()
            self.get_drop_op()
            self.get_conv_op()
            if self.encoding_operations is None:
                self.init_encoder()
            else:
                self.init_encoder_backbone()
        if self.encoder_only is not True and parent_class is False:
            self.init_upscale_ops()
            self.init_link_ops()
            self.init_decoder()
            self.init_final_layer()
            if self.bottleneck_classification is True:
                self.init_bottleneck_classifier()
            if self.feature_conditioning == 0:
                self.feature_conditioning = None
            if self.feature_conditioning is not None:
                self.init_feature_conditioning_operations()

    def get_norm_op(self):
        if self.norm_type is None:
            self.norm_op = torch.nn.Identity
            return
        self.norm_op = norm_fn_dict[self.norm_type][self.spatial_dimensions]

    def get_drop_op(self):
        if self.dropout_type is None:
            self.drop_op = torch.nn.Identity
        elif self.dropout_type == "dropout":
            self.drop_op = torch.nn.Dropout
        elif self.dropout_type == "uout":
            self.drop_op = UOut

    def get_conv_op(self):
        if self.spatial_dimensions not in (2, 3):
            raise ValueError("spatial_dimensions must be 2 or 3")
        if self.conv_type == "regular":
            self.conv_op_enc = self.conv_block
            self.conv_op_dec = self.conv_block
        elif self.conv_type == "depthwise":
            self.conv_op_enc = self.depthwise_conv_block
            self.conv_op_dec = self.depthwise_conv_block
        elif self.conv_type == "resnet":
# ... 44 lines not shown

    sae_2d = sae_block
    sae_3d = sae_block

    def asp_block(self, in_d, out_d, kernel_size, stride=None, padding=None):
        from ..layers.adn_fn import get_adn_fn
        from ..layers.multi_resolution import (AtrousSpatialPyramidPooling2d,
                                               AtrousSpatialPyramidPooling3d)
        asp = AtrousSpatialPyramidPooling3d if self.spatial_dimensions == 3 else AtrousSpatialPyramidPooling2d
        return asp(in_d, out_d, [1, 2],
                   get_adn_fn(self.spatial_dimensions, "instance", self.activation_fn, self.dropout_param))

    asp_2d = asp_block
    asp_3d = asp_block

    def res_block_conv_3d(self, in_d, out_d, kernel_size, stride=None, padding=None):
        nd = self.spatial_dimensions
        res, pool = (ResidualBlock3d, MaxPool3d) if nd == 3 else (ResidualBlock2d, MaxPool2d)
        inter_d = int(in_d) if in_d > 32 else None
        stride = _per_dim(1 if stride is None else stride, nd)
        block = res(in_d, kernel_size, inter_d, out_d, adn_fn=self.adn_fn)
        if any(s > 1 for s in stride):
            padding = _per_dim(0 if padding is None else padding, nd)
            new_padding = [p // 2 if p > s // 2 else p for p, s in zip(padding, stride)]
            return torch.nn.Sequential(block, pool(stride, stride, padding=new_padding))
        return block

    def adn_fn(self, s: int) -> torch.nn.Module:
        return ActDropNorm(in_channels=s, ordering="NDA", norm_fn=self.norm_op,
                           act_fn=self.activation_fn, dropout_fn=self.drop_op,
                           dropout_param=self.dropout_param)

    def init_upscale_ops(self):
        depths_a = self.depth[:0:-1]
        depths_b = self.depth[-2::-1]
        ops_ = []
        if self.upscale_type == "upsample":
            conv = Conv3d if self.spatial_dimensions == 3 else Conv2d
            for d1, d2, s in zip(depths_a, depths_b, self.strides[::-1][1:]):
                ops_.append(torch.nn.Sequential(conv(d1, d2, 1),
                                                Upsample(scale_factor=s, mode=self.interpolation)))
        elif self.upscale_type == "transpose":
            convt = ConvTranspose3d if self.spatial_dimensions == 3 else ConvTranspose2d
            for d1, d2, s in zip(depths_a, depths_b, self.strides[::-1][1:]):
                s = _per_dim(s, self.spatial_dimensions)
                p = [int(np.maximum(i - 2, 0)) for i in s]
                ops_.append(convt(d1, d2, s, stride=s, padding=p))
        self.upscale_ops = torch.nn.ModuleList(ops_)

    def init_link_ops(self):
        ex = self.skip_conditioning if self.skip_conditioning is not None else 0
        rev_depth = self.depth[-2::-1]
        if self.link_type == "identity":
            self.link_ops = torch.nn.ModuleList([torch.nn.Identity() for _ in self.depth[:-1]])
        elif self.link_type == "conv":
            self.link_ops = torch.nn.ModuleList([
                torch.nn.Sequential(self._conv(d + ex, d, 3, padding=self.padding), self.adn_fn(d))
                for d in rev_depth])
        elif self.link_type == "residual":
            block = ResidualBlock3d if self.spatial_dimensions == 3 else ResidualBlock2d
            self.link_ops = torch.nn.ModuleList([
                block(d + ex, 3, out_channels=d, adn_fn=self.adn_fn) for d in rev_depth])
        elif self.link_type == "attention":
            from ..layers.self_attention import SelfAttentionBlock
            self.link_ops = torch.nn.ModuleList([
                SelfAttentionBlock(self.spatial_dimensions, d, d, [16, 16, 1])
                for d in self.depth[-2::-1]])
        else:
            raise NotImplementedError(f"link_type={self.link_type!r} is outside the HIP path")

    def init_encoder(self):
        self.encoding_operations = self._build_encoder()

    def _build_encoder(self):
        encoding_operations = torch.nn.ModuleList([])
        previous_d = self.in_channels
        nd = self.spatial_dimensions
        k = None
        for i in range(len(self.depth) - 1):
            d = self.depth[i]
            k = _per_dim(self.kernel_sizes[i], nd)
            s = _per_dim(self.strides[i], nd)
            p = [int(j // 2) for j in k]
            op = torch.nn.Sequential(
                self.conv_op_enc(previous_d, d, kernel_size=k, stride=1, padding=self.padding),
                self.adn_fn(d))
            op_downsample = torch.nn.Sequential(
                self.conv_op_enc(d, d, kernel_size=k, stride=s, padding=p), self.adn_fn(d))
            encoding_operations.append(torch.nn.ModuleList([op, op_downsample]))
            previous_d = d
        op = torch.nn.Sequential(
            self.conv_op_enc(self.depth[-2], self.depth[-1], kernel_size=k, stride=1,
                             padding=self.padding),
            self.adn_fn(self.depth[-1]))
        encoding_operations.append(torch.nn.ModuleList([op, torch.nn.Identity()]))
        return encoding_operations

    def init_encoder_backbone(self):
        pool = MaxPool3d if self.spatial_dimensions == 3 else MaxPool2d
        for i in range(len(self.encoding_operations)):
            s = np.array(_per_dim(self.strides[i], self.spatial_dimensions))
            self.encoding_operations[i][1] = pool(kernel_size=tuple(int(j) for j in s),
                                                  stride=tuple(int(j) for j in s),
                                                  padding=tuple(int(j) for j in s // 2))
        self.encoding_operations[-1][1] = torch.nn.Identity()

    def init_decoder(self):
        self.decoding_operations = torch.nn.ModuleList([])
        depths = self.depth[-2::-1]
        kernel_sizes = self.kernel_sizes[-2::-1]
        self.deep_supervision_ops = torch.nn.ModuleList([])
        for d, k in zip(depths, kernel_sizes):
            k = _per_dim(k, self.spatial_dimensions)
            op = _DecoderOp(
                self.conv_op_dec(d * 2, d, kernel_size=k, stride=1, padding=self.padding),
                self.adn_fn(d))
            self.decoding_operations.append(op)
            if self.deep_supervision is True:
                self.deep_supervision_ops.append(self.get_ds_final_layer(d))

    def _head(self, d, padding):
        last = torch.nn.Softmax(dim=1) if self.n_classes > 2 else torch.nn.Sigmoid()
        nc = self.n_classes if self.n_classes > 2 else 1
        return torch.nn.Sequential(self._conv(d, d, 3, padding=padding), self.adn_fn(d),
                                   self._conv(d, nc, 1), last)

    def get_final_layer(self, d: int) -> torch.nn.Module:
        return self._head(d, "same")

    def get_ds_final_layer(self, d: int) -> torch.nn.Module:
        return self._head(d, 0)

    def init_final_layer(self):
        self.final_layer = self.get_final_layer(self.depth[0])

    def init_feature_conditioning_operations(self):
        depths = self.depth[-2::-1]
        self.feature_conditioning_ops = torch.nn.ModuleList([])
        if self.feature_conditioning_params is not None:
            self.f_mean = torch.nn.parameter.Parameter(
                self.feature_conditioning_params["mean"], requires_grad=False)
            self.f_std = torch.nn.parameter.Parameter(
                self.feature_conditioning_params["std"], requires_grad=False)
        else:
            self.f_mean = torch.nn.parameter.Parameter(
                torch.zeros([self.feature_conditioning]), requires_grad=False)
            self.f_std = torch.nn.parameter.Parameter(
                torch.ones([self.feature_conditioning]), requires_grad=False)
        for d in depths:
            self.feature_conditioning_ops.append(torch.nn.Sequential(
                Linear(self.feature_conditioning, d),
                get_adn_fn(1, "batch", "swish", self.dropout_param)(d),
                Linear(d, d),
                get_adn_fn(1, "batch", "sigmoid", self.dropout_param)(d)))

    def init_bottleneck_classifier(self):
        nc = self.n_classes if self.n_classes > 2 else 1
        self.bottleneck_classifier = Linear(self.depth[-1], nc)

    def _final(self, layer, X, return_logits):
        mods = list(layer)
        X = _run_rest(mods[:-1], X)
        if return_logits is True:
            return X
        if isinstance(mods[-1], torch.nn.Sigmoid):
            if X.dim() == 4:
                return HF.norm_drop_act(X.unsqueeze(2), act="sigmoid").squeeze(2)
# ... 263 lines not shown
```

adell_mri_amd/ops.py:

```python
import collections
import ctypes
import math
import os

import torch

from . import _lib
from ._lib import ACT_IDS, AdellHipError, ConvDesc, NormActDesc, check


class KernelTimer:

    def __init__(self, only=None):
        self.records = []
        self._agg = None
        self.only = None if only is None else set(only)
        self.active = True

    def start(self):
        e = torch.cuda.Event(enable_timing=True)
        e.record()
        return e

    def stop(self, name, flops, e0, tag=None, nbytes=0.0, kernels=1):
# ... 361 lines not shown
    N, Cout = dy.shape[:2]
    Cin = weight.shape[1]
    d = make_conv_desc(N, tuple(in_size), Cin, 0, Cout, tuple(weight.shape[2:]), 1, padding)
    assert (d.Do, d.Ho, d.Wo) == tuple(dy.shape[2:])
    dx = new_act(N, Cin, *in_size, dy.device)
    wc = weight.contiguous()
    check(_timed("adell_cin_small_kernel", _conv_flops(d),
                 lambda: _lib.lib().adell_conv_cin_small_bwd_data(
                     ctypes.byref(d), _ptr(dy), _ptr(wc), _ptr(dx), _stream()),
                 _conv_tag(d, "dgrad"), _conv_bytes(d)))
    return dx


def conv_cinfold_ok(weight, x0, x1, stride, padding, residual):
    if residual is not None or x1 is not None or weight.dim() != 5 or x0.dim() != 5:
        return False
    if FLAGS.get("no_cinfold") or x0.shape[1] > 4 or weight.shape[0] <= 4:
        return False
    return (tuple(weight.shape[2:]) == (3, 3, 3) and tuple(stride) == (1, 1, 1)
            and all(0 <= p <= 1 for p in padding))


def conv_cinfold_fwd(x, weight, bias, padding, want_stats, f16x3=False):
    _require_cuda(x, weight, bias)
    x = ndhwc(x)
    N, Cin, D, H, W = x.shape
    Cout = weight.shape[0]
    d = make_conv_desc(N, (D, H, W), Cin, 0, Cout, 3, 1, padding)
    y = new_act(N, Cout, d.Do, d.Ho, d.Wo, x.device)
    part = None
    wc = weight.contiguous()
    if want_stats:
        nt = _lib.lib().adell_conv_cinfold_ntiles(ctypes.byref(d))
        if nt < 0:
            check(nt)
        part = torch.empty((N, nt, Cout, 2), device=x.device, dtype=torch.float32)
    fn = _lib.lib().adell_conv_cinfold_fwd_f16x3 if f16x3 else _lib.lib().adell_conv_cinfold_fwd
    check(_timed("adell_cinfold_kernel", _conv_flops(d),
                 lambda: fn(ctypes.byref(d), _ptr(x), _ptr(wc), _ptr(bias), _ptr(y), _ptr(part),
                            0 if part is None else part.shape[1], _stream()),
                 _conv_tag(d, "fwd"), _conv_bytes(d)))
    return y, part


def conv_cinfold_bwd_weight(x, dy, padding, want_db, f16x3=False):
    _require_cuda(x, dy)
    x, dy = ndhwc(x), ndhwc(dy)
    N, Cin, D, H, W = x.shape
    Cout = dy.shape[1]
    d = make_conv_desc(N, (D, H, W), Cin, 0, Cout, 3, 1, padding)
    assert (d.Do, d.Ho, d.Wo) == tuple(dy.shape[2:])
    nbytes = _lib.lib().adell_conv_cinfold_wgrad_workspace(ctypes.byref(d))
    check(min(nbytes, 0))
    ws = _workspace(nbytes, x.device)
    dw = torch.empty((Cout, Cin, 3, 3, 3), device=x.device, dtype=torch.float32)
    db = torch.empty(Cout, device=x.device, dtype=torch.float32) if want_db else None
    fn = (_lib.lib().adell_conv_cinfold_bwd_weight_f16x3 if f16x3
          else _lib.lib().adell_conv_cinfold_bwd_weight)
    check(_timed("adell_cinfold_kernel", _conv_flops(d),
                 lambda: fn(ctypes.byref(d), _ptr(x), _ptr(dy), _ptr(dw), _ptr(db), _ptr(ws),
                            ws.numel() * 4, _stream()), _conv_tag(d, "wgrad"), _conv_bytes(d)))
    return dw, db


def conv_cinfold_bwd_data(dy, weight, in_size, padding, f16x3=False):
    _require_cuda(dy, weight)
    dy = ndhwc(dy)
    N, Cout = dy.shape[:2]
    Cin = weight.shape[1]
    d = make_conv_desc(N, tuple(in_size), Cin, 0, Cout, 3, 1, padding)
    assert (d.Do, d.Ho, d.Wo) == tuple(dy.shape[2:])
    if not _lib.lib().adell_conv_cinfold_dx_applicable(ctypes.byref(d)):
        return None
    dx = new_act(N, Cin, *in_size, dy.device)
    wc = weight.contiguous()
    fn = (_lib.lib().adell_conv_cinfold_bwd_data_f16x3 if f16x3
          else _lib.lib().adell_conv_cinfold_bwd_data)
    check(_timed("adell_cinfold_kernel", _conv_flops(d),
                 lambda: fn(ctypes.byref(d), _ptr(dy), _ptr(wc), _ptr(dx), _stream()),
                 _conv_tag(d, "dgrad"), _conv_bytes(d)))
    return dx


def conv1_small_ok(weight, Cin, stride, padding, residual):
    return (residual is None and weight.dim() == 5 and tuple(weight.shape[2:]) == (1, 1, 1)
            and weight.shape[0] <= 4 and Cin <= 512 and tuple(stride) == (1, 1, 1)
            and tuple(padding) == (0, 0, 0))


def _conv1_desc(N, size, C0, C1, Cout):
    return make_conv_desc(N, tuple(size), C0, C1, Cout, (1, 1, 1), (1, 1, 1), (0, 0, 0))


def conv1_small_fwd(x0, x1, weight, bias):
    _require_cuda(x0, x1, weight, bias)
    x0 = ndhwc(x0)
    N, C0, D, H, W = x0.shape
    C1 = 0
    if x1 is not None:
        x1 = ndhwc(x1)
        C1 = x1.shape[1]
    Cout = weight.shape[0]
    d = _conv1_desc(N, (D, H, W), C0, C1, Cout)
    y = new_act(N, Cout, D, H, W, x0.device)
    wc = weight.contiguous()
    check(_timed("adell_conv1_small_kernel", _conv_flops(d),
                 lambda: _lib.lib().adell_conv1_small_fwd(ctypes.byref(d), _ptr(x0), _ptr(x1),
                                                          _ptr(wc), _ptr(bias),
                                                          _ptr(y), _stream()),
                 _conv_tag(d, "fwd"), _conv_bytes(d)))
    return y


def conv1_small_bwd_data(dy, weight, in_size, C0, C1):
    dy = ndhwc(dy)
    N, Cout = dy.shape[:2]
    d = _conv1_desc(N, in_size, C0, C1, Cout)
    dx0 = new_act(N, C0, *in_size, dy.device)
    dx1 = new_act(N, C1, *in_size, dy.device) if C1 > 0 else None
    wc = weight.contiguous()
    check(_timed("adell_conv1_small_kernel", _conv_flops(d),
                 lambda: _lib.lib().adell_conv1_small_bwd_data(ctypes.byref(d), _ptr(dy),
                                                               _ptr(wc),
                                                               _ptr(dx0), _ptr(dx1), _stream()),
                 _conv_tag(d, "dgrad"), _conv_bytes(d)))
    return dx0, dx1


def conv1_small_bwd_weight(x0, x1, dy, want_db):
    x0, dy = ndhwc(x0), ndhwc(dy)
    N, C0, D, H, W = x0.shape
    C1 = 0
    if x1 is not None:
        x1 = ndhwc(x1)
        C1 = x1.shape[1]
    Cout = dy.shape[1]
    d = _conv1_desc(N, (D, H, W), C0, C1, Cout)
    ws = _workspace(_lib.lib().adell_conv1_small_wgrad_workspace(ctypes.byref(d)), x0.device)
    dw = torch.empty((Cout, C0 + C1, 1, 1, 1), device=x0.device, dtype=torch.float32)
    db = torch.empty((Cout,), device=x0.device, dtype=torch.float32) if want_db else None
    check(_timed("adell_conv1_small_kernel", _conv_flops(d),
                 lambda: _lib.lib().adell_conv1_small_bwd_weight(
                     ctypes.byref(d), _ptr(x0), _ptr(x1), _ptr(dy), _ptr(dw), _ptr(db), _ptr(ws),
                     ws.numel() * 4, _stream()), _conv_tag(d, "wgrad"), _conv_bytes(d)))
    return dw, db


def conv3d_bwd_data(dy, w_packed_bwd, in_size, C0, C1, kernel, stride, padding, amax=None,
                    add0=None):
    split = isinstance(w_packed_bwd, SplitWeight)
    if add0 is not None and split and C1 == 0:
        _require_cuda(dy, add0)
        dy, add0 = ndhwc(dy), ndhwc(add0)
        N, Cout = dy.shape[:2]
        d = make_conv_desc(N, tuple(in_size), C0, 0, Cout, kernel, stride, padding)
        dx0 = new_act(N, C0, *in_size, dy.device)
        ws, wsb = _splitk_workspace(d, 1, dy.device)
        check(_timed("adell_conv_igemm_f16_kernel", _conv_flops(d),
                     lambda: _lib.lib().adell_conv3d_bwd_data_f16x3_add(
                         ctypes.byref(d), _ptr(dy), _ptr(w_packed_bwd.halfs),
                         _ptr(w_packed_bwd.scale), _ptr(add0), _ptr(dx0), _ptr(amax), _ptr(ws), wsb,
                         _stream()), _conv_tag(d, "dgrad"), _conv_bytes(d, True)))
        return dx0, None
    _require_cuda(dy)
    dy = ndhwc(dy)
    N, Cout = dy.shape[:2]
# ... 496 lines not shown
    k, st = _triple(kernel), _triple(stride)
    if k != (3, 3, 3) or st != (1, 1, 1) or C0 % 16 or C1 % 16:
        return False
    d = make_conv_desc(N, tuple(in_size), C0, C1, Cout, kernel, stride, padding)
    return bool(_lib.lib().adell_conv3d_f16x3_rows_ok(ctypes.byref(d)))


def norm_act_fwd(x, mean, rstd, act, gamma=None, beta=None, act_w=None, act_p=0.0,
                 stats_per_item=1, drop_p=0.0, seed=0, rng_offset=0, want_mask=False,
                 split_exp=None):
    _require_cuda(x, mean, rstd, gamma, beta, act_w)
    x = ndhwc(x)
    d = make_na_desc(x, act, stats_per_item, act_p, 0 if act_w is None else act_w.numel(),
                     drop_p, seed, rng_offset)
    out = new_act(*x.shape, x.device)
    mask = None
    if want_mask and drop_p > 0.0:
        nbytes = _lib.lib().adell_norm_act_mask_bytes(ctypes.byref(d))
        if nbytes < 0:
            check(int(nbytes))
        mask = torch.empty((nbytes // 8,), device=x.device, dtype=torch.int64)
    if split_exp is not None:
        check(_timed(NORM_ACT_FAMILY, 0.0, lambda: _lib.lib().adell_norm_act_fwd_split(
            ctypes.byref(d), _ptr(x), _ptr(mean), _ptr(rstd), _ptr(gamma), _ptr(beta), _ptr(act_w),
            _ptr(out), int(split_exp), _ptr(mask), _stream()), "fwd", 8.0 * x.numel()))
    elif mask is not None:
        check(_timed(NORM_ACT_FAMILY, 0.0, lambda: _lib.lib().adell_norm_act_fwd_mask(
            ctypes.byref(d), _ptr(x), _ptr(mean), _ptr(rstd), _ptr(gamma), _ptr(beta), _ptr(act_w),
            _ptr(out), _ptr(mask), _stream()), "fwd", 8.0 * x.numel()))
    else:
        check(_timed(NORM_ACT_FAMILY, 0.0, lambda: _lib.lib().adell_norm_act_fwd(
            ctypes.byref(d), _ptr(x), _ptr(mean), _ptr(rstd), _ptr(gamma), _ptr(beta), _ptr(act_w),
            _ptr(out), _stream()), "fwd", 8.0 * x.numel()))
    return (out, mask) if want_mask else out


def norm_act_bwd_from_dt(x, dt, mean, rstd, partials, poff=0):
    _require_cuda(x, dt, mean, rstd, partials)
    x, dt = ndhwc(x), ndhwc(dt)
    d = make_na_desc(x, "identity", 1)
    N, C = x.shape[:2]
    ws = _workspace(4 * (2 + 2 * ((int(partials.shape[1]) + 255) // 256)) * N * C, x.device)
    check(_timed(NORM_ACT_FAMILY, 0.0, lambda: _lib.lib().adell_norm_act_bwd_from_dt(
        ctypes.byref(d), _ptr(x), _ptr(dt), _ptr(mean), _ptr(rstd), _ptr(partials),
        int(partials.shape[1]), int(partials.shape[2]), int(poff), _ptr(dt), _ptr(ws),
        ws.numel() * 4, _stream()), "bwd", 12.0 * x.numel()))
    return dt


def prelu_wgrad(x, dout, mean, rstd, act_w, gamma=None, beta=None, stats_per_item=1, drop_p=0.0,
                seed=0, rng_offset=0):
    _require_cuda(x, dout, mean, rstd, gamma, beta, act_w)
    x, dout = ndhwc(x), ndhwc(dout)
    d = make_na_desc(x, "prelu", stats_per_item, 0.0, act_w.numel(), drop_p, seed, rng_offset)
    ws = _workspace(_lib.lib().adell_prelu_wgrad_workspace(ctypes.byref(d)), x.device)
    dw = torch.empty_like(act_w)
    check(_lib.lib().adell_prelu_wgrad(ctypes.byref(d), _ptr(x), _ptr(dout), _ptr(mean), _ptr(rstd),
                                       _ptr(gamma), _ptr(beta), _ptr(dw), _ptr(ws),
                                       ws.numel() * 4, _stream()))
    return dw


def norm_act_bwd(x, dout, mean, rstd, act, gamma=None, beta=None, act_w=None, act_p=0.0,
                 stats_per_item=1, drop_p=0.0, seed=0, rng_offset=0, want_affine_grads=False):
    _require_cuda(x, dout, mean, rstd, gamma, beta, act_w)
    x, dout = ndhwc(x), ndhwc(dout)
    d = make_na_desc(x, act, stats_per_item, act_p, 0 if act_w is None else act_w.numel(),
                     drop_p, seed, rng_offset)
    dx = new_act(*x.shape, x.device)
    dgamma = dbeta = None
    if want_affine_grads:
        dgamma = torch.empty((x.shape[1],), device=x.device, dtype=torch.float32)
        dbeta = torch.empty_like(dgamma)
    ws = None
    if mean is not None or want_affine_grads:
        ws = _workspace(_lib.lib().adell_norm_act_bwd_workspace(ctypes.byref(d)), x.device)
    check(_timed(NORM_ACT_FAMILY, 0.0, lambda: _lib.lib().adell_norm_act_bwd(
        ctypes.byref(d), _ptr(x), _ptr(dout), _ptr(mean), _ptr(rstd), _ptr(gamma), _ptr(beta),
        _ptr(act_w), _ptr(dx), _ptr(dgamma), _ptr(dbeta), _ptr(ws),
        0 if ws is None else ws.numel() * 4, _stream()), "bwd", 12.0 * x.numel()))
    return dx, dgamma, dbeta


def norm_act_lowrank_ok(x, co):
    C = x.shape[1]
    return 1 <= co <= 4 and 4 <= C <= 1024 and (C & (C - 1)) == 0


def norm_act_bwd_lowrank(x, g, w, mean, rstd, act, act_p=0.0, drop_p=0.0, seed=0, rng_offset=0):
    _require_cuda(x, g, w, mean, rstd)
    x, g = ndhwc(x), ndhwc(g)
    co = g.shape[1]
    w = w.reshape(co, x.shape[1]).contiguous()
    assert g.shape[0] == x.shape[0] and g.shape[2:] == x.shape[2:]
    d = make_na_desc(x, act, 1, act_p, 0, drop_p, seed, rng_offset)
    dx = new_act(*x.shape, x.device)
    ws = _workspace(_lib.lib().adell_norm_act_bwd_workspace(ctypes.byref(d)), x.device)
    nb = 8.0 * x.numel() + 4.0 * g.numel()
    check(_timed(NORM_ACT_FAMILY, 0.0, lambda: _lib.lib().adell_norm_act_bwd_lowrank(
        ctypes.byref(d), _ptr(x), _ptr(g), _ptr(w), co, _ptr(mean), _ptr(rstd), _ptr(dx), _ptr(ws),
        ws.numel() * 4, _stream()), "bwd", nb))
    return dx


def dice_focal_fwd(prob, target, smooth, dice_eps, gamma, focal_eps, focal_alpha=1.0):
    _require_cuda(prob, target)
    prob, target = prob.contiguous(), target.contiguous()
    B = prob.shape[0]
    S = prob.numel() // B
    assert target.numel() == prob.numel()
    ws = _workspace(_lib.lib().adell_dice_focal_workspace(B, S), prob.device)
    dice = torch.empty((B,), device=prob.device, dtype=torch.float32)
    focal = torch.empty_like(dice)
    sums = torch.empty((B, 3), device=prob.device, dtype=torch.float32)
    check(_lib.lib().adell_dice_focal_fwd(_ptr(prob), _ptr(target), B, S, smooth, dice_eps, gamma,
                                          float(focal_alpha), focal_eps, _ptr(dice), _ptr(focal),
                                          _ptr(sums),
                                          _ptr(ws), ws.numel() * 4, _stream()))
    return dice, focal, sums


def dice_focal_bwd(prob, target, sums, smooth, dice_eps, gamma, focal_eps, gdice, gfocal,
                   focal_alpha=1.0):
    prob, target = prob.contiguous(), target.contiguous()
    B = prob.shape[0]
    S = prob.numel() // B
    dprob = torch.empty_like(prob)
    check(_lib.lib().adell_dice_focal_bwd(_ptr(prob), _ptr(target), B, S, smooth, dice_eps, gamma,
                                          float(focal_alpha), focal_eps, _ptr(sums), float(gdice),
                                          float(gfocal),
                                          _ptr(dprob), _stream()))
    return dprob


def dice_focal_bwd_dev(prob, target, sums, smooth, dice_eps, gamma, focal_eps, gdice, gfocal,
                       focal_alpha=1.0):
    prob, target = prob.contiguous(), target.contiguous()
    B = prob.shape[0]
    S = prob.numel() // B
    dprob = torch.empty_like(prob)
    gd = None if gdice is None else gdice.contiguous().float()
    gf = None if gfocal is None else gfocal.contiguous().float()
    check(_lib.lib().adell_dice_focal_bwd_dev(_ptr(prob), _ptr(target), B, S, smooth, dice_eps,
                                              gamma, float(focal_alpha), focal_eps, _ptr(sums),
                                              _ptr(gd), _ptr(gf), _ptr(dprob), _stream()))
    return dprob


def class_sums_fwd(p, t):
    _require_cuda(p, t)
    B, V, C = p.shape
    nbytes = _lib.lib().adell_class_sums_workspace(B, V, C)
    ws = _workspace(nbytes, p.device)
    sums = torch.empty((B, C, 3), device=p.device, dtype=torch.float32)
    check(_lib.lib().adell_class_sums_fwd(_ptr(p), _ptr(t), B, V, C, _ptr(sums), _ptr(ws),
                                          ws.numel() * 4, _stream()))
    return sums


def class_sums_bwd(t, gsums):
    _require_cuda(t, gsums)
    B, V, C = t.shape
    dp = torch.empty_like(t)
    g = gsums.contiguous()
    check(_lib.lib().adell_class_sums_bwd(_ptr(t), _ptr(g), B, V, C, _ptr(dp), _stream()))
    return dp
# ... 1056 lines not shown
```

include/adell_hip.h:

```cpp
#ifndef ADELL_HIP_H
#define ADELL_HIP_H

#include <stddef.h>
#include <stdint.h>

#ifdef __cplusplus
extern "C" {
#endif
#if defined(__GNUC__) || defined(__clang__)
#pragma GCC visibility push(default)
#endif

#define ADELL_OK 0
#define ADELL_E_BADARG (-1)
#define ADELL_E_UNSUPPORTED (-2)
#define ADELL_E_HIP (-3)
#define ADELL_E_NOMEM (-4)

#define ADELL_ABI_VERSION 2

enum {
  ADELL_ACT_IDENTITY = 0,
  ADELL_ACT_SILU = 1,
  ADELL_ACT_RELU = 2,
// ... 152 lines not shown
int adell_convtranspose3d_k2s2_fwd(int N, int D, int H, int W, int Cin, int Cout,
                                   const float* x, const float* w_packed,
                                   const float* bias, float* y, void* stream);
int adell_convtranspose3d_k2s2_bwd_data(int N, int D, int H, int W, int Cin,
                                        int Cout, const float* dy,
                                        const float* w_packed_bwd, float* dx,
                                        void* stream);
long adell_convtranspose3d_k2s2_bwd_weight_workspace(int N, int D, int H, int W,
                                                     int Cin, int Cout);
int adell_convtranspose3d_k2s2_bwd_weight(int N, int D, int H, int W, int Cin,
                                          int Cout, const float* x, const float* dy,
                                          float* dw, void* workspace,
                                          size_t workspace_bytes, void* stream);

long adell_stats_finalize_workspace(int N, int ntiles, int C);
int adell_stats_finalize(const float* partials, int N, int ntiles, int C,
                         long count, float eps, int per_item, float* mean,
                         float* rstd, void* workspace, size_t workspace_bytes,
                         void* stream);

int adell_bn_running_update(const float* mean, const float* rstd, float* running_mean,
                            float* running_var, long long* num_batches_tracked, int C, long count,
                            float eps, float momentum, void* stream);
int adell_bn_stats_sums(const float* partials, int N, int ntiles, int C, long count, double* sums,
                        void* workspace, size_t workspace_bytes, void* stream);
int adell_bn_stats_from_sums(const double* sums, int C, float eps, float* mean, float* rstd,
                             float* running_mean, float* running_var,
                             long long* num_batches_tracked, float momentum, void* stream);
int adell_channel_partials_ntiles(long V);
int adell_channel_partials(const float* x, int N, long V, int C, float* partials,
                           void* stream);

typedef struct adell_norm_act_desc {
  int64_t N, V;
  int32_t C;
  int32_t stats_per_item;
  int32_t act;
  int32_t act_w_n;
  float act_p;
  float drop_p;
  uint64_t seed;
  uint32_t rng_offset;
} adell_norm_act_desc;

int adell_norm_act_fwd(const adell_norm_act_desc* d, const float* x,
                       const float* mean, const float* rstd, const float* gamma,
                       const float* beta, const float* act_w, float* out,
                       void* stream);

long adell_norm_act_mask_bytes(const adell_norm_act_desc* d);
int adell_norm_act_fwd_mask(const adell_norm_act_desc* d, const float* x, const float* mean,
                            const float* rstd, const float* gamma, const float* beta,
                            const float* act_w, float* out, void* keep_mask, void* stream);
int adell_norm_act_fwd_split(const adell_norm_act_desc* d, const float* x, const float* mean,
                             const float* rstd, const float* gamma, const float* beta,
                             const float* act_w, void* out_rows, int split_exp, void* keep_mask,
                             void* stream);
int adell_split_rows_from_f32(const float* x, int N, long V, int C, const int* xk, void* rows,
                              void* stream);
int adell_split_rows_to_f32(const void* rows, int N, long V, int C, const int* xk, float* x,
                            void* stream);
int adell_norm_act_bwd_from_dt(const adell_norm_act_desc* d, const float* x, const float* dt,
                               const float* mean, const float* rstd, const float* partials,
                               int ntiles, int pstride, int poff, float* dx, void* workspace,
                               size_t workspace_bytes, void* stream);

long adell_norm_act_bwd_workspace(const adell_norm_act_desc* d);
int adell_norm_act_bwd(const adell_norm_act_desc* d, const float* x, const float* dout,
                       const float* mean, const float* rstd, const float* gamma,
                       const float* beta, const float* act_w, float* dx, float* dgamma,
                       float* dbeta, void* workspace, size_t workspace_bytes,
                       void* stream);
int adell_norm_act_bwd_sums(const adell_norm_act_desc* d, const float* x, const float* dout,
                            const float* mean, const float* rstd, const float* gamma,
                            const float* beta, const float* act_w, double* sums, float* dgamma,
                            float* dbeta, void* workspace, size_t workspace_bytes, void* stream);
int adell_norm_act_bwd_apply_sums(const adell_norm_act_desc* d, const float* x, const float* dout,
                                  const float* mean, const float* rstd, const float* gamma,
                                  const float* beta, const float* act_w, const double* sums,
                                  float* dx, void* workspace, size_t workspace_bytes, void* stream);
int adell_norm_act_bwd_lowrank(const adell_norm_act_desc* d, const float* x, const float* g,
                               const float* w, int co, const float* mean, const float* rstd,
                               float* dx, void* workspace, size_t workspace_bytes, void* stream);
long adell_prelu_wgrad_workspace(const adell_norm_act_desc* d);
int adell_prelu_wgrad(const adell_norm_act_desc* d, const float* x, const float* dout,
                      const float* mean, const float* rstd, const float* gamma, const float* beta,
                      float* dact_w, void* workspace, size_t workspace_bytes, void* stream);

long adell_dice_focal_workspace(int B, long S);
int adell_dice_focal_fwd(const float* prob, const float* target, int B, long S,
                         float smooth, float dice_eps, float gamma, float focal_alpha, float focal_eps,
                         float* dice, float* focal, float* sums, void* workspace,
                         size_t workspace_bytes, void* stream);
int adell_dice_focal_bwd(const float* prob, const float* target, int B, long S,
                         float smooth, float dice_eps, float gamma, float focal_alpha, float focal_eps,
                         const float* sums, float gdice, float gfocal, float* dprob,
                         void* stream);
int adell_dice_focal_bwd_dev(const float* prob, const float* target, int B, long S, float smooth,
                             float dice_eps, float gamma, float focal_alpha, float focal_eps,
                             const float* sums, const float* gdice, const float* gfocal,
                             float* dprob, void* stream);
long adell_class_sums_workspace(int B, long V, int C);
int adell_class_sums_fwd(const float* p, const float* t, int B, long V, int C, float* sums,
                         void* workspace, size_t workspace_bytes, void* stream);
int adell_class_sums_bwd(const float* t, const float* gsums, int B, long V, int C, float* dp,
                         void* stream);

int adell_sgd_step(float* param, const float* grad, float* momentum_buf, long n, float lr,
                   float momentum, float weight_decay, int nesterov, int first_step,
                   float grad_scale, void* stream);
int adell_adamw_step(float* param, const float* grad, float* exp_avg, float* exp_avg_sq,
                     long n, float lr, float beta1, float beta2, float eps,
                     float weight_decay, long step, float grad_scale, void* stream);
int adell_adam_step(float* param, const float* grad, float* exp_avg, float* exp_avg_sq, long n,
                    float lr, float beta1, float beta2, float eps, float weight_decay, long step,
                    float grad_scale, void* stream);

int adell_optim_step(int kind, float* param, const float* grad, float* state1, float* state2,
                     long n, float weight_decay, float eps, float grad_scale, const float* c5,
                     void* stream);
int adell_ema_update(float* shadow, const float* param, long n, float decay, void* stream);

int adell_layernorm_fwd(const float* x, const float* gamma, const float* beta, float* y,
                        float* mean, float* rstd, long rows, int C, float eps, void* stream);
long adell_layernorm_bwd_workspace(long rows, int C);
int adell_layernorm_bwd(const float* x, const float* dy, const float* gamma,
                        const float* mean, const float* rstd, float* dx, float* dgamma,
                        float* dbeta, long rows, int C, void* workspace,
                        size_t workspace_bytes, void* stream);
int adell_add_bcast(const float* a, const float* b, float* out, long n, long period,
                    void* stream);
int adell_sum_bcast(const float* g, float* db, long n, long period, void* stream);
int adell_attention_fwd(const float* q, const float* k, const float* v, const float* bias,
                        int nbias, int BH, int T, int A, int Dv, float scale, float drop_p,
                        unsigned long long seed, unsigned int rng_offset, float* out,
                        float* lse, void* stream);
int adell_attention_bwd(const float* q, const float* k, const float* v, const float* bias,
                        int nbias, const float* out, const float* dout, const float* lse,
                        int BH, int T, int A, int Dv, float scale, float drop_p,
                        unsigned long long seed, unsigned int rng_offset, float* dq, float* dk,
                        float* dv, void* stream);
#define ADELL_ATT_VALU 0
#define ADELL_ATT_MFMA_RESIDENT 1
#define ADELL_ATT_MFMA_STREAMED 2
#define ADELL_ATT_REFUSED 3
int adell_attention_plan(int pass, int T, int A, int Dv, int aligned, int* out);
int adell_attention_strided_ok(int T, int A, int Dv);
int adell_attention_fwd_strided(const float* q, const float* k, const float* v, const float* bias,
                                int nbias, int B, int H, int T, int A, int Dv, const long* strides,
                                float scale, float drop_p, unsigned long long seed,
                                unsigned int rng_offset, float* out, float* lse, void* stream);
int adell_attention_bwd_strided(const float* q, const float* k, const float* v, const float* bias,
                                int nbias, const float* out, const float* dout, const float* lse,
                                int B, int H, int T, int A, int Dv, const long* strides,
                                float scale, float drop_p, unsigned long long seed,
                                unsigned int rng_offset, float* dq, float* dk, float* dv,
                                void* stream);
int adell_attention_fwd_labels(const float* q, const float* k, const float* v, const float* bias,
                               int nbias, const int* labels, int nlab, int H, int BH, int T, int A,
                               int Dv, float scale, float drop_p, unsigned long long seed,
                               unsigned int rng_offset, float* out, float* lse, void* stream);
int adell_attention_bwd_labels(const float* q, const float* k, const float* v, const float* bias,
                               int nbias, const int* labels, int nlab, int H, const float* out,
                               const float* dout, const float* lse, int BH, int T, int A, int Dv,
                               float scale, float drop_p, unsigned long long seed,
                               unsigned int rng_offset, float* dq, float* dk, float* dv,
// ... 43 lines not shown
                    const float* acc, float* y, int N, long V, int C, void* stream);
long adell_cse_apply_bwd_workspace_floats(int N, long V, int C);
int adell_cse_apply_bwd(const float* x, const float* dy, const float* s, const float* c,
                        const float* inv, float* dx, float* ds, float* dc, int N, long V, int C,
                        float* workspace, void* stream);
int adell_bcast_nc(const float* g, float* out, int N, long V, int C, float scale, void* stream);

int adell_maxpool3d_fwd(const adell_conv3d_desc* d, const float* x, float* y,
                        int32_t* argmax, void* stream);
int adell_maxpool3d_bwd(const adell_conv3d_desc* d, const float* dy, const int32_t* argmax,
                        float* dx, void* stream);

int adell_dwconv3d_fwd(int N, int C, int D, int H, int W, int KD, int KH, int KW,
                       const float* x, const float* w, const float* bias, float* y,
                       void* stream);
int adell_dwconv3d_bwd_data(int N, int C, int D, int H, int W, int KD, int KH, int KW,
                            const float* dy, const float* w, float* dx, void* stream);
long adell_dwconv3d_bwd_weight_workspace_floats(int N, int C, int D, int H, int W, int KD, int KH,
                                                int KW);
int adell_dwconv3d_bwd_weight(int N, int C, int D, int H, int W, int KD, int KH, int KW,
                              const float* x, const float* dy, float* dw, float* db,
                              float* workspace, void* stream);
long adell_vicreg_scratch_floats(int B, int D);
int adell_vicreg_fwd(const float* x1, const float* x2, int B, int D, float min_var, float eps,
                     float* scratch, float* out3, void* stream);
int adell_vicreg_bwd(const float* x1, const float* x2, int B, int D, float min_var, float eps,
                     const float* scratch, const float* g3, float* dx1, float* dx2,
                     void* stream);

long adell_pair_loss_scratch_floats(int B, int D);
int adell_pair_loss_fwd(const float* x1, const float* x2, int B, int D, int kind,
                        float temperature, int apply_relu, float* scratch, float* loss,
                        void* stream);
int adell_pair_loss_bwd(const float* x1, const float* x2, int B, int D, int kind,
                        float temperature, int apply_relu, const float* scratch, const float* g,
                        float* dx1, float* dx2, void* stream);

long adell_loco_loss_workspace(int B, long S, int C);
int adell_loco_loss_fwd(const float* f1, const float* f2, int B, long S, int C, float temperature,
                        float eps, float* loss, void* workspace, size_t workspace_bytes,
                        void* stream);
int adell_loco_loss_bwd(const float* f1, const float* f2, const float* gloss, int B, long S, int C,
                        float temperature, float eps, float* df1, float* df2, void* stream);

int adell_convt_k2_applicable(int N, int D, int H, int W, int Cin, int Cout);
int adell_convt_k2_fwd(int N, int D, int H, int W, int Cin, int Cout, const float* x,
                       const float* w, const float* bias, float* y, void* stream);
int adell_convt_k2_bwd_data(int N, int D, int H, int W, int Cin, int Cout, const float* dy,
                            const float* w, float* dx, void* stream);
long adell_convt_k2_wgrad_workspace(int N, int D, int H, int W, int Cin, int Cout);
int adell_convt_k2_bwd_weight(int N, int D, int H, int W, int Cin, int Cout, const float* x,
                              const float* dy, float* dw, float* db, void* workspace,
                              size_t workspace_bytes, void* stream);
int adell_convt_k221_applicable(int N, int D, int H, int W, int Cin, int Cout);
int adell_convt_k221_fwd(int N, int D, int H, int W, int Cin, int Cout, const float* x,
                         const float* w, const float* bias, float* y, void* stream);
int adell_convt_k221_bwd_data(int N, int D, int H, int W, int Cin, int Cout, const float* dy,
                              const float* w, float* dx, void* stream);
long adell_convt_k221_wgrad_workspace(int N, int D, int H, int W, int Cin, int Cout);
int adell_convt_k221_bwd_weight(int N, int D, int H, int W, int Cin, int Cout, const float* x,
                                const float* dy, float* dw, float* db, void* workspace,
                                size_t workspace_bytes, void* stream);

int adell_conv_cinfold_applicable(const adell_conv3d_desc* d);
int adell_conv_cinfold_ntiles(const adell_conv3d_desc* d);
int adell_conv_cinfold_fwd(const adell_conv3d_desc* d, const float* x, const float* w,
                           const float* bias, float* y, float* stat_partials, int partial_rows,
                           void* stream);
int adell_conv_cinfold_fwd_f16x3(const adell_conv3d_desc* d, const float* x, const float* w,
                                 const float* bias, float* y, float* stat_partials, int partial_rows,
                           void* stream);
long adell_conv_cinfold_wgrad_workspace(const adell_conv3d_desc* d);
int adell_conv_cinfold_bwd_weight(const adell_conv3d_desc* d, const float* x, const float* dy,
                                  float* dw, float* db, void* workspace, size_t workspace_bytes,
                                  void* stream);
int adell_conv_cinfold_bwd_weight_f16x3(const adell_conv3d_desc* d, const float* x, const float* dy,
                                        float* dw, float* db, void* workspace,
                                        size_t workspace_bytes, void* stream);
int adell_conv_cinfold_dx_applicable(const adell_conv3d_desc* d);
int adell_conv_cinfold_bwd_data(const adell_conv3d_desc* d, const float* dy, const float* w,
                                float* dx, void* stream);
int adell_conv_cinfold_bwd_data_f16x3(const adell_conv3d_desc* d, const float* dy, const float* w,
                                      float* dx, void* stream);

int adell_conv1_small_applicable(const adell_conv3d_desc* d);
int adell_conv1_small_fwd(const adell_conv3d_desc* d, const float* x0, const float* x1,
                          const float* w, const float* bias, float* y, void* stream);
int adell_conv1_small_bwd_data(const adell_conv3d_desc* d, const float* dy, const float* w,
                               float* dx0, float* dx1, void* stream);
long adell_conv1_small_wgrad_workspace(const adell_conv3d_desc* d);
int adell_conv1_small_bwd_weight(const adell_conv3d_desc* d, const float* x0, const float* x1,
                                 const float* dy, float* dw, float* db, void* workspace,
                                 size_t workspace_bytes, void* stream);

int adell_conv_cin_small_applicable(const adell_conv3d_desc* d);
int adell_conv_cin_small_ntiles(const adell_conv3d_desc* d);
int adell_conv_cin_small_fwd(const adell_conv3d_desc* d, const float* x, const float* w,
                             const float* bias, float* y, float* stat_partials, int partial_rows,
                           void* stream);
int adell_conv_cin_small_bwd_data(const adell_conv3d_desc* d, const float* dy, const float* w,
                                  float* dx, void* stream);

int adell_multi_copy(const long* table, int rows, float* dst, void* stream);

long adell_grad_norm_workspace(int runs);
int adell_grad_norm_partials(const float* g, long n, int norm_inf, double* partials, int run,
                             void* stream);
int adell_grad_norm_finalize(const double* partials, int runs, int norm_inf, float scale,
                             float max_norm, float* out, void* stream);
int adell_grad_scale_by(float* g, long n, const float* coef_dev, void* stream);
int adell_multi_accumulate(const long* table, int rows, float* dst, void* stream);

enum { ADELL_SEG_IOU = 0, ADELL_SEG_PRECISION = 1, ADELL_SEG_FBETA = 2, ADELL_SEG_DICE = 3 };
long adell_seg_confusion_workspace(long n, int C);
int adell_seg_confusion_update(const float* pred, const void* target, int target_type, long B, int C,
                               long S, int channels_last, int* workspace, long workspace_bytes,
                               long long* const* states, int nstates, void* stream);
int adell_seg_metric_compute(const long long* state, int C, int kind, float beta, float* out,
                             void* stream);

long adell_cc_workspace(long NV, int D, int H, int W);
int adell_cc_label(const float* x, long NV, int D, int H, int W, int use_threshold, float threshold,
                   int* labels, int* counts, void* workspace, long workspace_bytes, void* stream);
long adell_picai_tables_workspace(long B, int D, int H, int W);
long adell_picai_tables_capacity(long B, int D, int H, int W);
int adell_picai_tables(const float* pred, const float* target, long B, int D, int H, int W,
                       int use_threshold, float threshold, int* hdr, int* out, long out_capacity,
                       void* workspace, long workspace_bytes, void* stream);

long adell_lesion_candidates_workspace(long NV, int D, int H, int W, int mode);
long adell_lesion_candidates_capacity(int D, int H, int W, int mode, int min_voxels, int num_lesions);
int adell_lesion_candidates(const float* x, long NV, int D, int H, int W, int mode, float threshold,
                            float factor, int min_voxels, int num_lesions, int round_decimals,
                            int use_round, int remove_adjacent, float* hard, int* indexed, int* n_out,
                            int* ids, float* conf, float* peak, long cap, int* rounds,
                            void* workspace, long workspace_bytes, void* stream);

int adell_gather_nd(const float* in, float* out, int nd, const int* sizes, const int* axis,
                    const long* mult, int na, const long* extent, const long* stride,
                    const long* shift, void* stream);
int adell_layernorm_rows_fwd(const float* x, long rows, int C, int inner, long so, long si,
                             const float* gamma, const float* beta, float eps, float* y,
                             float* mean, float* rstd, void* stream);
long adell_layernorm_rows_bwd_workspace(long rows, int C);
int adell_layernorm_rows_bwd(const float* x, const float* dy, const float* gamma,
                             const float* mean, const float* rstd, long rows, int C, int inner,
                             long so, long si, float* dx, long dso, long dsi, float* dgamma,
                             float* dbeta, void* workspace, size_t workspace_bytes, void* stream);
int adell_winattn_fwd(const float* q, const float* k, const float* v, long v_ts, long v_hs,
                      const float* rel, const float* mask, int n_mask, long W, int H, int T, int A,
                      int Dv, float scale, float drop_p, unsigned long seed, unsigned rng_offset,
                      float* out, float* lse, void* stream);
int adell_winattn_bwd(const float* q, const float* k, const float* v, long v_ts, long v_hs,
                      const float* rel, const float* mask, int n_mask, const float* o,
                      const float* dout, const float* lse, long W, int H, int T, int A, int Dv,
                      float scale, float drop_p, unsigned long seed, unsigned rng_offset,
                      float* dq, float* dk, float* dv, float* ds, void* stream);

long adell_gemm_f32_workspace_floats(int M, int N, int K);
int adell_gemm_f32(int M, int N, int K, const float* A, long lda, int a_kc, const float* B,
                   long ldb, int b_kc, float* C, long ldc, const float* bias,
                   const float* residual, long ldr, float* workspace, void* stream);

int adell_absmax_f32(const float* x, long n, uint32_t* out, void* stream);
int adell_gemm_f16x3_applicable(int M, int N, int K, const float* A, long lda, int a_kc,
                                const float* B, long ldb, int b_kc);
// ... 90 lines not shown
```

Baseline: 61.54 volumes/s.

## Fuse norm-act backward into first-layer cinfold conv dgrad and wgrad kernel

Adds a fused backward kernel for the first 3x3x3 conv (2->32 channels). It recomputes the instance-norm, activation and dropout backward per site while computing both data and weight gradients in a single pass with f16x3 MFMA. The norm-act backward is deferred through a placeholder/producer record, so the full 32-channel gradient tensor is never materialized and re-read. The cost is a considerably more complex autograd path: a separate constants kernel, only-reader tracking, and extra register/LDS pressure in the fused kernel.

```diff
diff --git a/adell_mri_amd/_lib.py b/adell_mri_amd/_lib.py
--- a/adell_mri_amd/_lib.py
+++ b/adell_mri_amd/_lib.py
@@ -202,6 +202,13 @@
     "adell_conv_cinfold_dx_applicable": (_i, [ctypes.POINTER(ConvDesc)]),
     "adell_conv_cinfold_bwd_data": (_i, [ctypes.POINTER(ConvDesc)] + [_vp] * 4),
     "adell_conv_cinfold_bwd_data_f16x3": (_i, [ctypes.POINTER(ConvDesc)] + [_vp] * 4),
+    "adell_conv_cinfold_bwd_site_applicable": (_i, [ctypes.POINTER(ConvDesc)]),
+    "adell_conv_cinfold_bwd_site_workspace": (_l, [ctypes.POINTER(ConvDesc)]),
+    "adell_conv_cinfold_bwd_site_f16x3": (_i, [ctypes.POINTER(ConvDesc)] + [_vp] * 6 + [_i, _f, _f, _vp,
+                                               ctypes.c_size_t] + [_vp] * 6
+                                          + [ctypes.c_size_t, _vp]),
+    "adell_norm_act_bwd_consts": (_i, [ctypes.POINTER(NormActDesc)] + [_vp] * 7
+                                  + [ctypes.c_size_t, _vp]),
     "adell_pair_loss_scratch_floats": (_l, [_i, _i]),
     "adell_pair_loss_fwd": (_i, [_vp, _vp, _i, _i, _i, _f, _i, _vp, _vp, _vp]),
     "adell_pair_loss_bwd": (_i, [_vp, _vp, _i, _i, _i, _f, _i, _vp, _vp, _vp, _vp, _vp]),
diff --git a/adell_mri_amd/csrc/conv_cinfold.hip b/adell_mri_amd/csrc/conv_cinfold.hip
--- a/adell_mri_amd/csrc/conv_cinfold.hip
+++ b/adell_mri_amd/csrc/conv_cinfold.hip
@@ -1243,3 +1243,450 @@
     default: return adell_cinfold_dx_launch<4>(a, grid, st, f16x3);
   }
 }
+
+#include "norm_act_site.h"
+
+struct CinFoldSiteArgs {
+  const float* g;
+  const float* y0;
+  const float* mean;
+  const float* rstd;
+  const float* c1;
+  const float* c2;
+  const unsigned long long* mask;
+  const float* x;
+  const float* w;
+  float* dx;
+  float* ws;
+  const unsigned* xmax;
+  long groups;
+  int N, D, H, W, Do, Ho, Wo, PD, PH, PW;
+  int ntx, nty, nseg, seglen;
+  int act;
+  float act_p, keep_scale;
+};
+
+constexpr int kCfsXCopy = 2 * 3 * 10 * 8;
+constexpr int kCfsLdsFloats = 2 * 128 * 16 + 128 * 65 + 8 + 2 * 64 * 16 + (6 * kCfsXCopy + 8) / 2 + 4 * 64 * 4;
+
+template <int ACT, bool DROP>
+__global__ __launch_bounds__(256, 2) void adell_cinfold_bwd_site_f16_kernel(CinFoldSiteArgs a) {
+  constexpr int CIN = 2, KT = 54, NTL = 2, KP = 64, NCH = 2, TS = KP + 1, PIECES = 4;
+  constexpr int XCOPY = kCfsXCopy;
+  extern __shared__ float smem[];
+  char* sdy = reinterpret_cast<char*>(smem);
+  float* sT = smem + NCH * 128 * 16;
+  float* smax = sT + 128 * TS;
+  char* dys = reinterpret_cast<char*>(smax + 8);
+  _Float16* xs = reinterpret_cast<_Float16*>(dys + 2 * 64 * 64);
+  const int tid = threadIdx.x, lane = tid & 63, wave = tid >> 6, li = lane & 31, lh = lane >> 5;
+  constexpr int act = ACT;
+  int t = blockIdx.x;
+  const int tx = t % a.ntx;
+  t /= a.ntx;
+  const int ty = t % a.nty, seg = t / a.nty;
+  const int nb = blockIdx.y;
+  const int x0 = tx * 8, y0 = ty * 8;
+  const int z_beg = seg * a.seglen;
+  const int z_end = (z_beg + a.seglen) < a.D ? (z_beg + a.seglen) : a.D;
+  cf_half8 bh[NTL][NCH];
+  cf_half8* wlo = reinterpret_cast<cf_half8*>(xs + 6 * XCOPY + 8);
+  float wun[NTL];
+#pragma unroll
+  for (int nt = 0; nt < NTL; ++nt) {
+    const int k = nt * 32 + li;
+    const int tap = k < KT ? k / CIN : 0, ci = k < KT ? k - tap * CIN : 0;
+    float wv[NCH][8];
+    float mx = 0.f;
+#pragma unroll
+    for (int c = 0; c < NCH; ++c)
+#pragma unroll
+      for (int q = 0; q < 8; ++q) {
+        const int co = 16 * c + 8 * lh + q;
+        const float v = a.w[((size_t)co * CIN + ci) * 27 + tap];
+        wv[c][q] = k < KT ? v : 0.f;
+        mx = fmaxf(mx, fabsf(wv[c][q]));
+      }
+    mx = fmaxf(mx, __shfl_xor(mx, 32, 64));
+    const int kw = cf_scale_exp(mx);
+    const float wsc = __int_as_float((kw + 127) << 23);
+    wun[nt] = __int_as_float((127 - kw) << 23);
+#pragma unroll
+    for (int c = 0; c < NCH; ++c) {
+      cf_half8 lo;
+#pragma unroll
+      for (int q = 0; q < 8; ++q) {
+        const float v = wv[c][q] * wsc;
+        const _Float16 h = (_Float16)v;
+        bh[nt][c][q] = h;
+        lo[q] = (_Float16)(v - (float)h);
+      }
+      if (wave == 0) wlo[(nt * NCH + c) * 64 + lane] = lo;
+    }
+  }
+  const int kX = adell_cf_exp(__uint_as_float(a.xmax[0]));
+  const float sX = __int_as_float((kX + 127) << 23);
+  int boff[NTL], bkz[NTL];
+#pragma unroll
+  for (int nt = 0; nt < NTL; ++nt) {
+    const int k = nt * 32 + li;
+    if (k < KT) {
+      const int tap = k / CIN, ci = k - tap * CIN;
+      const int kz = tap / 9, ky = (tap - 9 * kz) / 3, kx = tap - 9 * kz - 3 * ky;
+      boff[nt] = ((kx * CIN + ci) * 30 + ky) * 8;
+      bkz[nt] = kz;
+    } else {
+      boff[nt] = -1;
+      bkz[nt] = 0;
+    }
+  }
+  const int cg = (lane >> 4) & 1, tq = (lane >> 2) & 3, tp = lane & 3;
+  const int abase = (lh * 8 + tq) * 64 + (16 * cg + 4 * tp) * 2 + wave * 16 * 64;
+  f32x16 accw[NTL];
+#pragma unroll
+  for (int nt = 0; nt < NTL; ++nt)
+#pragma unroll
+    for (int r = 0; r < 16; ++r) accw[nt][r] = 0.f;
+  float4 dbacc = make_float4(0.f, 0.f, 0.f, 0.f);
+  int kprev = 0;
+  bool first = true;
+  const int c4 = tid & 7;
+  const bool norm = a.mean != nullptr;
+  float sm[4], sr[4], sc1[4], sc2[4];
+#pragma unroll
+  for (int q = 0; q < 4; ++q) {
+    const int si = nb * 32 + 4 * c4 + q;
+    sm[q] = norm ? a.mean[si] : 0.f;
+    sr[q] = norm ? a.rstd[si] : 1.f;
+    sc1[q] = norm ? a.c1[si] : 0.f;
+    sc2[q] = norm ? a.c2[si] : 0.f;
+  }
+  auto own = [&](int u) -> int {
+    const int r = (tid >> 3) + 32 * u;
+    const int hy = r / 10, hx = r - hy * 10;
+    const int vy = hy - 2 + a.PH, vx = hx - 2 + a.PW;
+    return (r < 100 && vy >= 0 && vy < 8 && vx >= 0 && vx < 8) ? vy * 8 + vx : -1;
+  };
+  float4 gq[PIECES], yq[PIECES];
+  unsigned mk[DROP ? PIECES : 1][4];
+  unsigned okm = 0;
+  auto fetch_plane = [&](int p) {
+    okm = 0;
+#pragma unroll
+    for (int u = 0; u < PIECES; ++u) {
+      const int r = (tid >> 3) + 32 * u;
+      const int hy = r / 10, hx = r - hy * 10;
+      const int yy = y0 + a.PH - 2 + hy, xx = x0 + a.PW - 2 + hx;
+      const bool ok = r < 100 && p >= 0 && p < a.Do && yy >= 0 && yy < a.Ho && xx >= 0 && xx < a.Wo;
+      const size_t vox = ok ? (((size_t)p * a.Ho + yy) * a.Wo + xx) : 0;
+      const size_t off = ((size_t)nb * a.Do * a.Ho * a.Wo + vox) * 32 + 4 * c4;
+      gq[u] = *reinterpret_cast<const float4*>(a.g + off);
+      yq[u] = *reinterpret_cast<const float4*>(a.y0 + off);
+      if constexpr (DROP) {
+#pragma unroll
+        for (int q = 0; q < 4; ++q) mk[u][q] = adell_na_keep_half(a.mask, nb, a.groups, (long)vox * 8 + c4, q);
+      }
+      okm |= ok ? (1u << u) : 0u;
+    }
+  };
+  auto site_plane = [&](int p, int slot) {
+    float mx = 0.f;
+#pragma unroll
+    for (int u = 0; u < PIECES; ++u) {
+      const float gs[4] = {gq[u].x, gq[u].y, gq[u].z, gq[u].w};
+      const float ys[4] = {yq[u].x, yq[u].y, yq[u].z, yq[u].w};
+      float o[4];
+      long jj = 0;
+      if constexpr (DROP) {
+        const int r = (tid >> 3) + 32 * u;
+        const int hy = r / 10, hx = r - hy * 10;
+        const int yy = y0 + a.PH - 2 + hy, xx = x0 + a.PW - 2 + hx;
+        jj = (((long)p * a.Ho + yy) * a.Wo + xx) * 8 + c4;
+      }
+#pragma unroll
+      for (int q = 0; q < 4; ++q) {
+        bool keep = true;
+        if constexpr (DROP) keep = adell_na_keep_bit(mk[u][q], jj);
+        float hn;
+        const float dt = adell_na_site_dt(act, ys[q], gs[q], keep, a.keep_scale, sm[q], sr[q], 1.f,
+                                          0.f, a.act_p, &hn);
+        const float v = adell_na_site_dx(dt, hn, sr[q], 1.f, sc1[q], sc2[q], norm);
+        o[q] = ((okm >> u) & 1u) ? v : 0.f;
+        mx = fmaxf(mx, fabsf(o[q]));
+      }
+      gq[u] = make_float4(o[0], o[1], o[2], o[3]);
+    }
+#pragma unroll
+    for (int o = 32; o > 0; o >>= 1) mx = fmaxf(mx, __shfl_xor(mx, o, 64));
+    if (lane == 0) smax[slot * 4 + wave] = mx;
+  };
+  auto put_plane = [&](float sc, bool ownp) {
+#pragma unroll
+    for (int u = 0; u < PIECES; ++u) {
+      const int r = (tid >> 3) + 32 * u;
+      if (r < 100) {
+        const float v[4] = {gq[u].x * sc, gq[u].y * sc, gq[u].z * sc, gq[u].w * sc};
+        cf_half4 h, l;
+#pragma unroll
+        for (int q = 0; q < 4; ++q) {
+          h[q] = (_Float16)v[q];
+          l[q] = (_Float16)(v[q] - (float)h[q]);
+        }
+        const int sw = (r >> 2) & 3, slot = (c4 & 3) >> 1;
+        char* row = sdy + ((size_t)(c4 >> 2) * 128 + r) * 64 + (c4 & 1) * 8;
+        *reinterpret_cast<cf_half4*>(row + ((slot ^ sw) << 4)) = h;
+        *reinterpret_cast<cf_half4*>(row + (((2 + slot) ^ sw) << 4)) = l;
+        const int ov = own(u);
+        if (ownp && ov >= 0) {
+          *reinterpret_cast<cf_half4*>(dys + ov * 64 + c4 * 8) = h;
+          *reinterpret_cast<cf_half4*>(dys + 64 * 64 + ov * 64 + c4 * 8) = l;
+          dbacc.x += gq[u].x; dbacc.y += gq[u].y; dbacc.z += gq[u].z; dbacc.w += gq[u].w;
+        }
+      }
+    }
+  };
+  float2 xpre = make_float2(0.f, 0.f);
+  auto fetch_x = [&](int z) {
+    const int hy = tid / 10, hx = tid - hy * 10;
+    const int xx = x0 - a.PW + hx, yy = y0 - a.PH + hy;
+    const bool ok = tid < 100 && z >= 0 && z < a.D && yy >= 0 && yy < a.H && xx >= 0 && xx < a.W;
+    const size_t off = ok ? ((((size_t)nb * a.D + z) * a.H + yy) * a.W + xx) * 2 : 0;
+    const float2 f = *reinterpret_cast<const float2*>(a.x + off);
+    xpre = ok ? f : make_float2(0.f, 0.f);
+  };
+  auto put_x = [&](int slot) {
+    if (tid < 100) {
+      const int hy = tid / 10, hx = tid - hy * 10;
+      const float v[2] = {xpre.x * sX, xpre.y * sX};
+#pragma unroll
+      for (int ci = 0; ci < 2; ++ci) {
+        const _Float16 h = (_Float16)v[ci], l = (_Float16)(v[ci] - (float)h);
+#pragma unroll
+        for (int sh = 0; sh < 3; ++sh) {
+          const int xq = hx - sh;
+          if (xq >= 0 && xq < 8) {
+            const int o = (((sh * CIN + ci) * 3 + slot) * 10 + hy) * 8 + xq;
+            xs[o] = h;
+            xs[3 * XCOPY + o] = l;
+          }
+        }
+      }
+    }
+  };
+  for (int i = tid; i < NCH * 28 * 16; i += 256) {
+    const int c = i / (28 * 16), w = i - c * 28 * 16;
+    reinterpret_cast<float*>(sdy)[(c * 128 + 100) * 16 + w] = 0.f;
+  }
+  if (tid < 8) xs[6 * XCOPY + tid] = (_Float16)0.f;
+  const int p_first = z_beg + a.PD - 2, p_last = z_end - 1 + a.PD;
+  fetch_x(p_first - a.PD);
+  put_x(0);
+  fetch_x(p_first - a.PD + 1);
+  put_x(1);
+  fetch_x(p_first - a.PD + 2);
+  float run[3] = {0.f, 0.f, 0.f};
+  fetch_plane(p_first);
+  int it = 0, it3 = 0;
+  for (int p = p_first; p <= p_last; ++p, ++it, it3 = it3 == 2 ? 0 : it3 + 1) {
+    site_plane(p, it & 1);
+    __syncthreads();
+    const float* smp = smax + (it & 1) * 4;
+    const float pmax = fmaxf(fmaxf(smp[0], smp[1]), fmaxf(smp[2], smp[3]));
+    const int kd = cf_scale_exp(pmax);
+    const bool ownp = p >= z_beg && p < z_end && p < a.Do && pmax > 0.f;
+    put_plane(__int_as_float((kd + 127) << 23), ownp);
+    put_x(it3 == 0 ? 2 : it3 - 1);
+    __syncthreads();
+    if (p + 1 <= p_last) {
+      fetch_plane(p + 1);
+      fetch_x(p + 1 - a.PD + 2);
+    }
+    f32x16 acc[NTL];
+#pragma unroll
+    for (int nt = 0; nt < NTL; ++nt)
+#pragma unroll
+      for (int r = 0; r < 16; ++r) acc[nt][r] = 0.f;
+    const int rowi = wave * 32 + li;
+    const int sw = (rowi >> 2) & 3;
+#pragma unroll
+    for (int c = 0; c < NCH; ++c) {
+      const char* row = sdy + ((size_t)c * 128 + rowi) * 64;
+      const cf_half8 ah = *reinterpret_cast<const cf_half8*>(row + ((lh ^ sw) << 4));
+      const cf_half8 al = *reinterpret_cast<const cf_half8*>(row + (((2 + lh) ^ sw) << 4));
+#pragma unroll
+      for (int nt = 0; nt < NTL; ++nt) {
+        acc[nt] = __builtin_amdgcn_mfma_f32_32x32x16_f16(al, bh[nt][c], acc[nt], 0, 0, 0);
+        acc[nt] = __builtin_amdgcn_mfma_f32_32x32x16_f16(ah, wlo[(nt * NCH + c) * 64 + lane], acc[nt], 0, 0, 0);
+        acc[nt] = __builtin_amdgcn_mfma_f32_32x32x16_f16(ah, bh[nt][c], acc[nt], 0, 0, 0);
+      }
+    }
+    if (ownp) {
+      const int ksum = kX + kd;
+      if (!first && ksum != kprev) {
+#pragma unroll
+        for (int nt = 0; nt < NTL; ++nt)
+#pragma unroll
+          for (int r = 0; r < 16; ++r) accw[nt][r] = ldexpf(accw[nt][r], ksum - kprev);
+      }
+      kprev = ksum;
+      first = false;
+      const cf_half8 ah = adell_cf_trfrag(dys + abase);
+      const cf_half8 al = adell_cf_trfrag(dys + 64 * 64 + abase);
+#pragma unroll
+      for (int nt = 0; nt < NTL; ++nt) {
+        int zs = it3 + bkz[nt];
+        zs = zs >= 3 ? zs - 3 : zs;
+        const int o = boff[nt] + zs * 80 + (2 * wave + lh) * 8;
+        const _Float16* ph = boff[nt] >= 0 ? xs + o : xs + 6 * XCOPY;
+        const _Float16* pl = boff[nt] >= 0 ? xs + 3 * XCOPY + o : xs + 6 * XCOPY;
+        const cf_half8 xh8 = *reinterpret_cast<const cf_half8*>(ph);
+        const cf_half8 xl8 = *reinterpret_cast<const cf_half8*>(pl);
+        accw[nt] = __builtin_amdgcn_mfma_f32_32x32x16_f16(al, xh8, accw[nt], 0, 0, 0);
+        accw[nt] = __builtin_amdgcn_mfma_f32_32x32x16_f16(ah, xl8, accw[nt], 0, 0, 0);
+        accw[nt] = __builtin_amdgcn_mfma_f32_32x32x16_f16(ah, xh8, accw[nt], 0, 0, 0);
+      }
+    }
+    const float dun = __int_as_float((127 - kd) << 23);
+#pragma unroll
+    for (int nt = 0; nt < NTL; ++nt)
+#pragma unroll
+      for (int r = 0; r < 16; ++r) {
+        const int row = wave * 32 + (r & 3) + 8 * (r >> 2) + 4 * lh;
+        sT[row * TS + nt * 32 + li] = acc[nt][r] * (dun * wun[nt]);
+      }
+    __syncthreads();
+    if (tid < 64 * CIN) {
+      const int ci = tid % CIN, v = tid / CIN, vy = v >> 3, vx = v & 7;
+#pragma unroll
+      for (int kz = 0; kz < 3; ++kz) {
+        float t9 = 0.f;
+#pragma unroll
+        for (int ky = 0; ky < 3; ++ky)
+#pragma unroll
+          for (int kx = 0; kx < 3; ++kx) {
+            const int r = (vy + 2 - ky) * 10 + (vx + 2 - kx);
+            t9 += sT[r * TS + ((kz * 3 + ky) * 3 + kx) * CIN + ci];
+          }
+        run[kz] += t9;
+      }
+      const int z = p - a.PD, yy = y0 + vy, xx = x0 + vx;
+      if (z >= z_beg && z < z_end && yy < a.H && xx < a.W)
+        a.dx[((((size_t)nb * a.D + z) * a.H + yy) * a.W + xx) * CIN + ci] = run[0];
+      run[0] = run[1];
+      run[1] = run[2];
+      run[2] = 0.f;
+    }
+  }
+  __syncthreads();
+  float (*red)[KP + 1] = reinterpret_cast<float (*)[KP + 1]>(sT);
+  float* dbs = sT + 32 * (KP + 1);
+  dbs[tid * 4 + 0] = dbacc.x; dbs[tid * 4 + 1] = dbacc.y;
+  dbs[tid * 4 + 2] = dbacc.z; dbs[tid * 4 + 3] = dbacc.w;
+  for (int w = 0; w < 4; ++w) {
+    if (wave == w) {
+#pragma unroll
+      for (int nt = 0; nt < NTL; ++nt)
+#pragma unroll
+        for (int r = 0; r < 16; ++r) {
+          const int row = (r & 3) + 8 * (r >> 2) + 4 * lh;
+          float* q = &red[row][nt * 32 + li];
+          const float v = first ? 0.f : ldexpf(accw[nt][r], -kprev);
+          *q = w == 0 ? v : *q + v;
+        }
+    }
+    __syncthreads();
+  }
+  if (tid < 32) {
+    float s = 0.f;
+    for (int j = 0; j < 32; ++j) s += dbs[(j * 8 + (tid >> 2)) * 4 + (tid & 3)];
+    red[tid][KP] = s;
+  }
+  __syncthreads();
+  float* out = a.ws + ((size_t)blockIdx.y * gridDim.x + blockIdx.x) * 32 * (KP + 1);
+  for (int i = tid; i < 32 * (KP + 1); i += 256) out[i] = (&red[0][0])[i];
+}
+
+extern "C" int adell_conv_cinfold_bwd_site_applicable(const adell_conv3d_desc* d) {
+  return (adell_conv_cinfold_dx_applicable(d) && d->C0 == 2 && d->Cout == 32) ? 1 : 0;
+}
+
+static void adell_cinfold_site_grid(const adell_conv3d_desc* d, CinFoldSiteArgs* a) {
+  a->ntx = adell_cdiv(d->W, 8);
+  a->nty = adell_cdiv(d->H, 8);
+  const long cols = (long)a->ntx * a->nty * d->N;
+  int nseg = (int)((512 + cols - 1) / cols);
+  if (nseg < 1) nseg = 1;
+  while (nseg > 1 && adell_cdiv(d->D, nseg) < 8) --nseg;
+  a->seglen = adell_cdiv(d->D, nseg);
+  a->nseg = adell_cdiv(d->D, a->seglen);
+}
+
+extern "C" long adell_conv_cinfold_bwd_site_workspace(const adell_conv3d_desc* d) {
+  if (!adell_conv_cinfold_bwd_site_applicable(d)) return ADELL_E_BADARG;
+  CinFoldSiteArgs a = {};
+  adell_cinfold_site_grid(d, &a);
+  const long blocks = (long)a.ntx * a.nty * a.nseg * d->N;
+  return (long)sizeof(float) * (blocks * 32 * 65 + 4);
+}
+
+template <int ACT>
+static int adell_cinfold_site_launch(const CinFoldSiteArgs& a, dim3 grid, hipStream_t st) {
+  const size_t lds = (size_t)kCfsLdsFloats * sizeof(float);
+  if (a.mask) return adell_launch<adell_cinfold_bwd_site_f16_kernel<ACT, true>>(grid, dim3(256), lds, st, a);
+  return adell_launch<adell_cinfold_bwd_site_f16_kernel<ACT, false>>(grid, dim3(256), lds, st, a);
+}
+
+extern "C" int adell_conv_cinfold_bwd_site_f16x3(
+    const adell_conv3d_desc* d, const float* g, const float* y0, const float* mean,
+    const float* rstd, const float* c1, const float* c2, int act, float act_p, float keep_scale,
+    const void* keep_bits, size_t keep_bits_bytes, const float* x, const float* w, float* dx,
+    float* dw, float* db, void* workspace, size_t workspace_bytes, void* stream) {
+  ADELL_REQUIRE(g && y0 && x && w && dx && dw && workspace && adell_conv_cinfold_bwd_site_applicable(d),
+                "conv_cinfold_bwd_site_f16x3: 3x3x3 stride-1 conv 2 -> 32 expected");
+  ADELL_REQUIRE((mean == nullptr) == (rstd == nullptr) && (mean == nullptr) == (c1 == nullptr) &&
+                    (mean == nullptr) == (c2 == nullptr),
+                "conv_cinfold_bwd_site_f16x3: mean / rstd / c1 / c2 come together");
+  ADELL_REQUIRE(act == ADELL_ACT_IDENTITY || act == ADELL_ACT_SILU || act == ADELL_ACT_RELU ||
+                    act == ADELL_ACT_LEAKY_RELU,
+                "conv_cinfold_bwd_site_f16x3: identity, swish, relu or leaky relu expected");
+  ADELL_REQUIRE(((((uintptr_t)g | (uintptr_t)y0) & 15) == 0) && (((uintptr_t)x & 7) == 0),
+                "conv_cinfold_bwd_site_f16x3: g / y0 16-byte, x 8-byte aligned");
+  ADELL_REQUIRE((long)workspace_bytes >= adell_conv_cinfold_bwd_site_workspace(d),
+                "conv_cinfold_bwd_site_f16x3: workspace too small");
+  CinFoldSiteArgs a = {};
+  adell_cinfold_site_grid(d, &a);
+  a.g = g; a.y0 = y0; a.mean = mean; a.rstd = rstd; a.c1 = c1; a.c2 = c2;
+  a.mask = (const unsigned long long*)keep_bits;
+  a.x = x; a.w = w; a.dx = dx; a.ws = (float*)workspace;
+  a.N = d->N; a.D = d->D; a.H = d->H; a.W = d->W;
+  a.Do = d->Do; a.Ho = d->Ho; a.Wo = d->Wo; a.PD = d->PD; a.PH = d->PH; a.PW = d->PW;
+  a.act = act; a.act_p = act_p; a.keep_scale = keep_bits ? keep_scale : 1.0f;
+  const long vc = (long)d->Do * d->Ho * d->Wo * 32;
+  a.groups = (vc + 255) / 256;
+  ADELL_REQUIRE(!keep_bits || (long)keep_bits_bytes >= (long)d->N * a.groups * 32,
+                "conv_cinfold_bwd_site_f16x3: keep-bit buffer too small");
+  const long blocks = (long)a.ntx * a.nty * a.nseg * d->N;
+  ADELL_REQUIRE(blocks < 0x7fffffffL, "conv_cinfold_bwd_site_f16x3: too many blocks");
+  unsigned* xmax = reinterpret_cast<unsigned*>(a.ws + (size_t)blocks * 32 * 65);
+  a.xmax = xmax;
+  hipStream_t st = (hipStream_t)stream;
+  ADELL_CHECK_HIP(hipMemsetAsync(xmax, 0, 4 * sizeof(unsigned), st));
+  const long nx = (long)d->N * d->D * d->H * d->W * 2;
+  long ab = (nx / 4 + 1023) / 1024;
+  if (ab > 512) ab = 512;
+  if (ab < 1) ab = 1;
+  hipLaunchKernelGGL(adell_cinfold_absmax_kernel, dim3((unsigned)ab), dim3(256), 0, st, x, nx, xmax);
+  dim3 grid((unsigned)(a.ntx * a.nty * a.nseg), (unsigned)d->N);
+  int rc;
+  switch (act) {
+    case ADELL_ACT_SILU: rc = adell_cinfold_site_launch<ADELL_ACT_SILU>(a, grid, st); break;
+    case ADELL_ACT_RELU: rc = adell_cinfold_site_launch<ADELL_ACT_RELU>(a, grid, st); break;
+    case ADELL_ACT_LEAKY_RELU: rc = adell_cinfold_site_launch<ADELL_ACT_LEAKY_RELU>(a, grid, st); break;
+    default: rc = adell_cinfold_site_launch<ADELL_ACT_IDENTITY>(a, grid, st); break;
+  }
+  if (rc != ADELL_OK) return rc;
+  hipLaunchKernelGGL(adell_cinfold_wgrad_reduce_kernel, dim3(adell_cdiv(32 * 55, 4)), dim3(256), 0, st,
+                     (const float*)workspace, (int)blocks, 1, 64, 2, 32, dw, db);
+  ADELL_CHECK_HIP(hipGetLastError());
+  return ADELL_OK;
+}
diff --git a/adell_mri_amd/csrc/norm_act.hip b/adell_mri_amd/csrc/norm_act.hip
--- a/adell_mri_amd/csrc/norm_act.hip
+++ b/adell_mri_amd/csrc/norm_act.hip
@@ -1,4 +1,5 @@
 #include "common.h"
+#include "norm_act_site.h"
 
 ADELL_RNG_STEP_DEFINE(norm_act)
 
@@ -997,6 +998,32 @@
   return ADELL_OK;
 }
 
+extern "C" int adell_norm_act_bwd_consts(const adell_norm_act_desc* d, const float* x,
+                                         const float* dout, const float* mean, const float* rstd,
+                                         float* c1, float* c2, void* workspace,
+                                         size_t workspace_bytes, void* stream) {
+  NormActBwdArgs a = {};
+  int rc = adell_nab_fill(&a, d);
+  if (rc != ADELL_OK) return rc;
+  ADELL_REQUIRE(x && dout && mean && rstd && c1 && c2, "norm_act_bwd_consts: null pointer");
+  ADELL_REQUIRE(d->stats_per_item && d->N <= 65535 && d->act_w_n == 0,
+                "norm_act_bwd_consts: per-item statistics without activation weights expected");
+  ADELL_REQUIRE(workspace && (long)workspace_bytes >= adell_norm_act_bwd_workspace(d),
+                "norm_act_bwd_consts: workspace too small");
+  a.lr_shift = adell_ilog2(d->C) - 2;
+  a.x = x; a.dout = dout; a.mean = mean; a.rstd = rstd; a.dx = const_cast<float*>(x);
+  a.part = (float*)workspace;
+  bool vec, fast;
+  adell_na_bwd_route(a, d, &vec, &fast);
+  hipStream_t st = (hipStream_t)stream;
+  adell_na_bwd_partials_launch(a, d, fast, vec, st);
+  hipLaunchKernelGGL(adell_na_bwd_finalize_item_kernel, dim3(adell_cdiv(d->C, 8), (unsigned)d->N),
+                     dim3(256), 0, st, (const float*)a.part, a.ntiles, d->C, (double)d->V,
+                     (const float*)nullptr, c1, c2, d->C, 0);
+  ADELL_CHECK_HIP(hipGetLastError());
+  return ADELL_OK;
+}
+
 struct NaConst {
   float m[4], r[4], g[4], b[4], p[4], c1[4], c2[4];
 };
@@ -1147,14 +1174,10 @@
       float o[4];
 #pragma unroll
       for (int q = 0; q < 4; ++q) {
-        const float hn = (xs[q] - k.m[q]) * k.r[q];
-        const float t = hn * k.g[q] + k.b[q];
-        const float uu = keep[q] ? t * keep_scale : 0.f;
-        const float du = gs[q] * adell_act_grad(ACT, uu, k.p[q]);
-        const float dt = keep[q] ? du * keep_scale : 0.f;
-        float r = dt * k.g[q];
-        if (norm) r = k.r[q] * (r - k.c1[q] - hn * k.c2[q]);
-        o[q] = r;
+        float hn;
+        const float dt = adell_na_site_dt(ACT, xs[q], gs[q], keep[q], keep_scale, k.m[q], k.r[q],
+                                          k.g[q], k.b[q], k.p[q], &hn);
+        o[q] = adell_na_site_dx(dt, hn, k.r[q], k.g[q], k.c1[q], k.c2[q], norm);
       }
       dxo[jj] = make_float4(o[0], o[1], o[2], o[3]);
     }
@@ -1195,11 +1218,9 @@
       adell_na_keep4(a, (long)n * n4 + jj, keep);
 #pragma unroll
       for (int q = 0; q < 4; ++q) {
-        const float hn = (xs[q] - k.m[q]) * k.r[q];
-        const float t = hn * k.g[q] + k.b[q];
-        const float uu = keep[q] ? t * keep_scale : 0.f;
-        const float du = gs[q] * adell_act_grad(ACT, uu, k.p[q]);
-        const float dt = keep[q] ? du * keep_scale : 0.f;
+        float hn;
+        const float dt = adell_na_site_dt(ACT, xs[q], gs[q], keep[q], keep_scale, k.m[q], k.r[q],
+                                          k.g[q], k.b[q], k.p[q], &hn);
         A[q] += dt;
         B[q] += dt * hn;
       }
diff --git a/adell_mri_amd/csrc/norm_act_site.h b/adell_mri_amd/csrc/norm_act_site.h
--- /dev/null
+++ b/adell_mri_amd/csrc/norm_act_site.h
@@ -0,0 +1,29 @@
+#pragma once
+#include "common.h"
+
+__device__ __forceinline__ float adell_na_site_dt(int act, float x, float dout, bool keep,
+                                                  float keep_scale, float mean, float rstd,
+                                                  float gamma, float beta, float pa, float* hn) {
+  const float h = (x - mean) * rstd;
+  const float t = h * gamma + beta;
+  const float uu = keep ? t * keep_scale : 0.f;
+  const float du = dout * adell_act_grad(act, uu, pa);
+  *hn = h;
+  return keep ? du * keep_scale : 0.f;
+}
+
+__device__ __forceinline__ float adell_na_site_dx(float dt, float hn, float rstd, float gamma,
+                                                  float c1, float c2, bool norm) {
+  float r = dt * gamma;
+  if (norm) r = rstd * (r - c1 - hn * c2);
+  return r;
+}
+
+__device__ __forceinline__ unsigned adell_na_keep_half(const unsigned long long* mask, long n,
+                                                       long groups, long jj, int q) {
+  const unsigned* m32 = reinterpret_cast<const unsigned*>(mask);
+  return m32[((n * groups + (jj >> 6)) * 4 + q) * 2 + ((jj >> 5) & 1)];
+}
+__device__ __forceinline__ bool adell_na_keep_bit(unsigned half, long jj) {
+  return (half >> (jj & 31)) & 1u;
+}
diff --git a/adell_mri_amd/functional.py b/adell_mri_amd/functional.py
--- a/adell_mri_amd/functional.py
+++ b/adell_mri_amd/functional.py
@@ -22,7 +22,8 @@
          "no_seq_attention": bool(os.environ.get("ADELL_NO_SEQ_ATTENTION")),
          "no_mlp_fuse": not bool(os.environ.get("ADELL_MLP_FUSE")),
          "mlp_min_elems": int(os.environ.get("ADELL_MLP_MIN_ELEMS", str(1 << 20))),
-         "no_cinfold_wgrad_f16": bool(os.environ.get("ADELL_NO_CINFOLD_WGRAD_F16"))}
+         "no_cinfold_wgrad_f16": bool(os.environ.get("ADELL_NO_CINFOLD_WGRAD_F16")),
+         "no_cinfold_bwd_fuse": bool(os.environ.get("ADELL_NO_CINFOLD_BWD_FUSE"))}
 
 
 def set_conv_precision(mode):
@@ -409,7 +410,7 @@
     @staticmethod
     def forward(ctx, x0, x1, weight, bias, residual, wp, conf):
         (stride, padding, want_stats, wref, ctx.carry_in, ctx.carry_out, ctx.carry_x0,
-         ctx.carry_cat, ctx.adn, rows0, rows1) = conf
+         ctx.carry_cat, ctx.adn, rows0, rows1, ctx.producer) = conf
         if (rows0 is not None or rows1 is not None) and not isinstance(wp, ops.SplitWeight):
             ops.ROWS_FALLBACKS[0] += 1
             if rows0 is not None:
@@ -487,6 +488,23 @@
             _side_ok(wref.obj)
             add0 = ctx.carry_in.take() if ctx.carry_in is not None else None
             return (add0 if need[0] else None), None, None, None, None, None, None
+        rec = ctx.producer.take() if ctx.producer is not None else None
+        if rec is not None:
+            if (dy.data_ptr() == rec.placeholder.data_ptr() and not any(dy.stride())
+                    and CONV_PRECISION == "f16x3"):
+                _side_ok(wref.obj, ctx.bias_ref.obj)
+                dx0, dw, db = ops.conv_cinfold_bwd_site(
+                    x0, weight, rec.g, rec.y0, rec.mean, rec.rstd, rec.c12, rec.act, padding,
+                    act_p=rec.act_p, drop_p=rec.drop_p, mask=rec.mask,
+                    want_db=has_bias and need[3])
+                add0 = ctx.carry_in.take() if ctx.carry_in is not None else None
+                if add0 is not None:
+                    dx0 = dx0 + add0
+                dx0, _ = _park_input_grads(ctx, dx0, None)
+                return dx0, None, (dw if need[2] else None), db, None, None, None
+            dsite = ops.norm_act_bwd(rec.y0, rec.g, rec.mean, rec.rstd, rec.act, act_p=rec.act_p,
+                                     drop_p=rec.drop_p, seed=rec.seed, rng_offset=rec.offset)[0]
+            dy = dsite if not any(dy.stride()) else dsite + ops.ndhwc(dy)
         dy = ops.ndhwc(dy)
         dx0 = dx1 = dw = db = dres = None
         add0 = ctx.carry_in.take() if ctx.carry_in is not None else None
@@ -645,6 +663,34 @@
         return g
 
 
+class SiteRecord:
+
+    __slots__ = ("g", "y0", "mean", "rstd", "c12", "mask", "drop_p", "seed", "offset", "act",
+                 "act_p", "placeholder")
+
+    def __init__(self, **kw):
+        for k, v in kw.items():
+            setattr(self, k, v)
+
+
+class ConvProducer:
+
+    __slots__ = ("record",)
+
+    def __init__(self):
+        self.record = None
+
+    def take(self):
+        r, self.record = self.record, None
+        return r
+
+
+def only_reader(t):
+    if t is not None and getattr(t, "_adell_producer", None) is not None:
+        t._adell_only_reader = True
+    return t
+
+
 class AdnSite:
 
     __slots__ = ("x", "mean", "rstd", "mask", "drop_p", "act", "act_p", "fused", "part", "poff",
@@ -706,7 +752,7 @@
     rows0 = getattr(x0, "_adell_rows", None)
     rows1 = getattr(x1, "_adell_rows", None) if x1 is not None else None
     conf = (stride, padding, want_stats, _Ref(weight), carry_in, carry_out, carry_x0, carry_cat,
-            adn, rows0, rows1)
+            adn, rows0, rows1, None)
     Cin = x0.shape[1] + (0 if x1 is None else x1.shape[1])
     small1 = ops.conv1_small_ok(weight, Cin, stride, padding, residual)
     if small1:
@@ -721,6 +767,11 @@
         wp = "cin_small"
     elif ops.conv_cinfold_ok(weight, x0, x1, stride, padding, residual):
         wp = "cinfold"
+        if (CONV_PRECISION == "f16x3" and not FLAGS["no_cinfold_bwd_fuse"]
+                and torch.is_grad_enabled() and x0.requires_grad and weight.requires_grad
+                and ops.conv_cinfold_bwd_site_ok(x0.shape[0], tuple(x0.shape[2:]), x0.shape[1],
+                                                 weight.shape[0], padding)):
+            conf = conf[:11] + (ConvProducer(),)
     elif (CONV_PRECISION == "f16x3" and x1 is None and weight.dim() == 5 and x0.shape[1] <= 4
           and 3 <= weight.shape[4] and weight.shape[4] * x0.shape[1] <= 16
           and stride == (1, 1, 1) and not FLAGS["no_fold"]):
@@ -730,6 +781,8 @@
     y, part = _Conv3dFn.apply(x0, x1, weight, bias, residual, wp, conf)
     if want_stats and part.numel() > 0:
         y._adell_partials = part
+    if conf[11] is not None:
+        y._adell_producer = conf[11]
     return y
 
 
@@ -791,7 +844,7 @@
 class _NormDropActFn(torch.autograd.Function):
     @staticmethod
     def forward(ctx, x, mean, rstd, gamma, beta, act_w, conf):
-        act, act_p, per_item, drop_p, seed, offset, site, split_exp, _group = conf
+        act, act_p, per_item, drop_p, seed, offset, site, split_exp, _group, _prod = conf
         if site is not None:
             out, mask = ops.norm_act_fwd(x, mean, rstd, act, gamma=gamma, beta=beta, act_w=act_w,
                                          act_p=act_p, stats_per_item=per_item, drop_p=drop_p,
@@ -809,7 +862,8 @@
     @staticmethod
     def backward(ctx, dout):
         x, mean, rstd, gamma, beta, act_w = ctx.saved_tensors
-        act, act_p, per_item, drop_p, seed, offset, site, _split_exp, group = ctx.conf
+        act, act_p, per_item, drop_p, seed, offset, site, _split_exp, group, prod = ctx.conf
+        mask = site.mask if site is not None else None
         if site is not None:
             fused, part, poff = site.fused, site.part, site.poff
             site.fused, site.part = False, None
@@ -823,6 +877,16 @@
             if fused:
                 dx = ops.norm_act_bwd_from_dt(x, ops.ndhwc(dout), mean, rstd, part, poff)
                 return dx, None, None, None, None, None, None
+        if (prod is not None and not FLAGS["no_cinfold_bwd_fuse"] and not grad_observed(x)
+                and not any(s == 0 and n > 1 for s, n in zip(dout.stride(), dout.shape))):
+            g = ops.ndhwc(dout)
+            c12 = ops.norm_act_bwd_consts(x, g, mean, rstd, act, act_p=act_p, drop_p=drop_p,
+                                          seed=seed, rng_offset=offset)
+            ph = dout.new_zeros(()).expand(x.shape)
+            prod.record = SiteRecord(g=g, y0=x, mean=mean, rstd=rstd, c12=c12, mask=mask,
+                                     drop_p=drop_p, seed=seed, offset=offset, act=act,
+                                     act_p=act_p, placeholder=ph)
+            return ph, None, None, None, None, None, None
         dact_w = None
         if act_w is not None and ctx.needs_input_grad[5]:
             dact_w = ops.prelu_wgrad(x, dout, mean, rstd, act_w, gamma=gamma, beta=beta,
@@ -853,6 +917,9 @@
                   momentum=0.1, act="identity", act_p=0.0, act_w=None, drop_p=0.0,
                   training=False, rows_reader=None, sync_group=None):
     part = getattr(x, "_adell_partials", None)
+    prod = getattr(x, "_adell_producer", None) if getattr(x, "_adell_only_reader", False) else None
+    if prod is not None and (grad_observed(x) or ops.ndhwc(x) is not x):
+        prod = None
     x = ops.ndhwc(x)
     N, C = x.shape[:2]
     V = x.shape[2] * x.shape[3] * x.shape[4]
@@ -900,7 +967,13 @@
             and ops.norm_act_mask_ok(x)):
         site = AdnSite(None, None, None, None, p, act, float(act_p))
     split_exp = _rows_exponent(x, rows_reader, norm, gamma, beta, act, float(act_p), act_w, p)
-    conf = (act, float(act_p), per_item, p, seed, offset, site, split_exp, group)
+    if prod is not None and not (
+            norm == "instance" and gamma is None and beta is None and act_w is None
+            and act in ops.SITE_BWD_ACTS and x.requires_grad and torch.is_grad_enabled()
+            and CONV_PRECISION == "f16x3" and not FLAGS["no_cinfold_bwd_fuse"]
+            and (p == 0.0 or site is not None)):
+        prod = None
+    conf = (act, float(act_p), per_item, p, seed, offset, site, split_exp, group, prod)
     out = _NormDropActFn.apply(x, mean, rstd, gamma, beta, act_w, conf)
     if site is not None:
         out._adell_site = site
diff --git a/adell_mri_amd/modules/segmentation/unet.py b/adell_mri_amd/modules/segmentation/unet.py
--- a/adell_mri_amd/modules/segmentation/unet.py
+++ b/adell_mri_amd/modules/segmentation/unet.py
@@ -92,6 +92,16 @@
     def forward(self, X, X_cat=None, carry_cat=None):
         h = self[0](X, X_cat=X_cat, carry_cat=carry_cat) if X_cat is not None else self[0](X)
         return self[1](h)
+
+
+class _EncoderOp(torch.nn.Sequential):
+
+    def forward(self, X):
+        mods = list(self)
+        h = HF.only_reader(mods[0](X))
+        for mod in mods[1:]:
+            h = mod(h)
+        return h
 
 
 class _DecoderOp(torch.nn.Sequential):
@@ -302,7 +312,7 @@
             k = _per_dim(self.kernel_sizes[i], nd)
             s = _per_dim(self.strides[i], nd)
             p = [int(j // 2) for j in k]
-            op = torch.nn.Sequential(
+            op = _EncoderOp(
                 self.conv_op_enc(previous_d, d, kernel_size=k, stride=1, padding=self.padding),
                 self.adn_fn(d))
             op_downsample = torch.nn.Sequential(
diff --git a/adell_mri_amd/ops.py b/adell_mri_amd/ops.py
--- a/adell_mri_amd/ops.py
+++ b/adell_mri_amd/ops.py
@@ -467,6 +467,50 @@
     return dx
 
 
+SITE_BWD_ACTS = ("identity", "swish", "silu", "relu", "leaky_relu")
+
+
+def conv_cinfold_bwd_site_ok(N, in_size, Cin, Cout, padding):
+    d = make_conv_desc(N, tuple(in_size), Cin, 0, Cout, 3, 1, padding)
+    return bool(_lib.lib().adell_conv_cinfold_bwd_site_applicable(ctypes.byref(d)))
+
+
+def conv_cinfold_bwd_site(x, weight, g, y0, mean, rstd, c12, act, padding, act_p=0.0, drop_p=0.0,
+                          mask=None, want_db=True):
+    _require_cuda(x, weight, g, y0, mean, rstd, c12)
+    x, g, y0 = ndhwc(x), ndhwc(g), ndhwc(y0)
+    N, Cin, D, H, W = x.shape
+    Cout = y0.shape[1]
+    d = make_conv_desc(N, (D, H, W), Cin, 0, Cout, 3, 1, padding)
+    assert (d.Do, d.Ho, d.Wo) == tuple(y0.shape[2:]) and g.shape == y0.shape
+    if (drop_p > 0.0) != (mask is not None):
+        raise _lib.AdellHipError("conv_cinfold_bwd_site: keep bits go with drop_p > 0")
+    nbytes = _lib.lib().adell_conv_cinfold_bwd_site_workspace(ctypes.byref(d))
+    check(min(nbytes, 0))
+    ws = _workspace(nbytes, x.device)
+    dx = new_act(N, Cin, D, H, W, x.device)
+    dw = torch.empty((Cout, Cin, 3, 3, 3), device=x.device, dtype=torch.float32)
+    db = torch.empty(Cout, device=x.device, dtype=torch.float32) if want_db else None
+    wc = weight.contiguous()
+    c1 = c2 = None
+    if mean is not None:
+        assert tuple(c12.shape) == (2, N, Cout) and c12.is_contiguous()
+        c1, c2 = c12[0], c12[1]
+    act_id = ACT_IDS[act] if isinstance(act, str) else int(act)
+    mptr = None if mask is None else ctypes.c_void_p(mask.data_ptr())
+    f32 = lambda v: ctypes.c_float(v).value
+    keep_scale = f32(1.0 / f32(1.0 - f32(drop_p)))
+    mbytes = 0 if mask is None else mask.numel() * mask.element_size()
+    nb = 4.0 * (g.numel() + y0.numel() + x.numel() + dx.numel())
+    check(_timed("adell_cinfold_kernel", 2.0 * _conv_flops(d),
+                 lambda: _lib.lib().adell_conv_cinfold_bwd_site_f16x3(
+                     ctypes.byref(d), _ptr(g), _ptr(y0), _ptr(mean), _ptr(rstd), _ptr(c1), _ptr(c2),
+                     act_id, float(act_p), keep_scale, mptr, mbytes, _ptr(x),
+                     _ptr(wc), _ptr(dx), _ptr(dw), _ptr(db), _ptr(ws), ws.numel() * 4, _stream()),
+                 _conv_tag(d, "bwd_site"), nb))
+    return dx, dw, db
+
+
 def conv1_small_ok(weight, Cin, stride, padding, residual):
     return (residual is None and weight.dim() == 5 and tuple(weight.shape[2:]) == (1, 1, 1)
             and weight.shape[0] <= 4 and Cin <= 512 and tuple(stride) == (1, 1, 1)
@@ -1129,6 +1173,19 @@
     return dx, dgamma, dbeta
 
 
+def norm_act_bwd_consts(x, dout, mean, rstd, act, act_p=0.0, drop_p=0.0, seed=0, rng_offset=0):
+    _require_cuda(x, dout, mean, rstd)
+    x, dout = ndhwc(x), ndhwc(dout)
+    N, C = x.shape[:2]
+    d = make_na_desc(x, act, 1, act_p, 0, drop_p, seed, rng_offset)
+    c12 = torch.empty((2, N, C), device=x.device, dtype=torch.float32)
+    ws = _workspace(_lib.lib().adell_norm_act_bwd_workspace(ctypes.byref(d)), x.device)
+    check(_timed(NORM_ACT_FAMILY, 0.0, lambda: _lib.lib().adell_norm_act_bwd_consts(
+        ctypes.byref(d), _ptr(x), _ptr(dout), _ptr(mean), _ptr(rstd), _ptr(c12[0]), _ptr(c12[1]),
+        _ptr(ws), ws.numel() * 4, _stream()), "bwd_consts", 8.0 * x.numel()))
+    return c12
+
+
 def norm_act_lowrank_ok(x, co):
     C = x.shape[1]
     return 1 <= co <= 4 and 4 <= C <= 1024 and (C & (C - 1)) == 0
diff --git a/include/adell_hip.h b/include/adell_hip.h
--- a/include/adell_hip.h
+++ b/include/adell_hip.h
@@ -258,6 +258,9 @@
 int adell_norm_act_bwd_lowrank(const adell_norm_act_desc* d, const float* x, const float* g,
                                const float* w, int co, const float* mean, const float* rstd,
                                float* dx, void* workspace, size_t workspace_bytes, void* stream);
+int adell_norm_act_bwd_consts(const adell_norm_act_desc* d, const float* x, const float* dout,
+                              const float* mean, const float* rstd, float* c1, float* c2,
+                              void* workspace, size_t workspace_bytes, void* stream);
 long adell_prelu_wgrad_workspace(const adell_norm_act_desc* d);
 int adell_prelu_wgrad(const adell_norm_act_desc* d, const float* x, const float* dout,
                       const float* mean, const float* rstd, const float* gamma, const float* beta,
@@ -467,6 +470,14 @@
                                 float* dx, void* stream);
 int adell_conv_cinfold_bwd_data_f16x3(const adell_conv3d_desc* d, const float* dy, const float* w,
                                       float* dx, void* stream);
+int adell_conv_cinfold_bwd_site_applicable(const adell_conv3d_desc* d);
+long adell_conv_cinfold_bwd_site_workspace(const adell_conv3d_desc* d);
+int adell_conv_cinfold_bwd_site_f16x3(const adell_conv3d_desc* d, const float* g, const float* y0,
+                                      const float* mean, const float* rstd, const float* c1,
+                                      const float* c2, int act, float act_p, float keep_scale,
+                                      const void* keep_bits, size_t keep_bits_bytes, const float* x,
+                                      const float* w, float* dx, float* dw, float* db,
+                                      void* workspace, size_t workspace_bytes, void* stream);
 
 int adell_conv1_small_applicable(const adell_conv3d_desc* d);
 int adell_conv1_small_fwd(const adell_conv3d_desc* d, const float* x0, const float* x1,
```

Result: slower. 60.81 volumes/s (-1.2%).
